# wildminder/ComfyUI-KEEP

Measured on AMD Instinct MI355X. Metric: restored 512x512 face frames/sec, T=20 clip, higher is better.
Workload: dtype f16x3; 1 GPU; 48 independent clips x T=20 x 512x512 per GPU (BASELINE configs[1] clips), KEEP config, synthetic weights seed 0, precision policy x3; clips_per_gpu=48, clip_length=20, parallelism=dp1 over clips, precision_policy=x3

## Files before the change

comfyui-keep_amd/csrc/keep_attn.hip:

```cpp
#include <math.h>
#include <stdlib.h>

#include <type_traits>

#include "keep_common.h"
#include "../../include/keep_cv_hip.h"

static constexpr int KEEP_NT_ATTN_O = 0;


struct AttnP {
  const float* q;
  const float* k;
  const float* v;
  const unsigned short* q16;
  const unsigned short* k16;
  const unsigned short* v16;
  float* o;
  long q_bs, q_ts, q_hs, k_bs, k_ts, k_hs, v_bs, v_ts, v_hs, o_bs, o_ts, o_hs;
  int B, H, Lq, Lk, D, Dv;
  float scale;
  int mode, T, seg_len;
  int img_h, img_w, ksplit, shift, kv_rot, n_img;
  int nslices;
  unsigned flags;
  const _Float16* kv_pack;
  const float* q_amax;
  const float* k_amax;
  const float* v_amax;
};

enum AttnForm {
  ATTN_F32,
  ATTN_BF16,
  ATTN_BF16IN,
  ATTN_X3_NQ8,
  ATTN_X3_NQ16,
  ATTN_X3_NQ0,
  ATTN_X3_PACKED,
  ATTN_X1_PACKED,
  ATTN_X3_SMALL,
  ATTN_X3_TWO_PASS,
  ATTN_X3_SFULL,
  ATTN_X3_SFULL2,
};
struct AttnPlan {
  AttnForm form;
  int waves;
  int dvt;
  bool masked;
  size_t lds;
  int64_t scratch;
  int nq;
  bool win_tables;
};

__device__ __forceinline__ void attn_range_scale(float amax, float& s, float& inv_s) {
  int e = (int)((__float_as_uint(amax) >> 23) & 0xffu);
  if (!(amax > 0.f) || e == 255) {
    s = 1.f;
    inv_s = 1.f;
    return;
  }
  e = e < 15 ? 15 : e;
  s = __uint_as_float((unsigned)(268 - e) << 23);
  inv_s = __uint_as_float((unsigned)(e - 14) << 23);
}

__device__ __forceinline__ void win_shift(const AttnP& p, int wh, int ww, int& sy, int& sx) {
  sy = p.shift > 0 ? wh / 2 : 0;
  sx = p.shift > 0 ? ww / 2 : 0;
}

__device__ __forceinline__ void win_decode(const AttnP& p, int bw, int t, int rot, int& img, int& pix) {
  const int k2 = p.ksplit * p.ksplit;
  img = bw / k2;
  const int widx = bw - img * k2;
  const int wy = widx / p.ksplit, wx = widx - wy * p.ksplit;
  const int wh = p.img_h / p.ksplit, ww = p.img_w / p.ksplit;
  int sy, sx;
  win_shift(p, wh, ww, sy, sx);
  const int ty = (int)(((float)t + 0.5f) * (1.0f / (float)ww)), tx = t - ty * ww;
  int y = wy * wh + ty + sy;
  int x = wx * ww + tx + sx;
  if (y >= p.img_h) y -= p.img_h;
  if (x >= p.img_w) x -= p.img_w;
  pix = y * p.img_w + x;
  if (rot) {
    img += rot;
    if (img >= p.n_img) img -= p.n_img;
  }
}
// ... 416 lines not shown
    l_run = l_run * alpha + lsum;
    m_run = m_new;

#pragma unroll
    for (int r = 0; r < 16; ++r) {
      const int qrow = (r & 3) + 8 * (r >> 2) + 4 * lhi;
      const float ar = __shfl(alpha, qrow);
#pragma unroll
      for (int j = 0; j < DVT; ++j) o[j][r] *= ar;
    }
#pragma unroll
    for (int st = 0; st < 2; ++st) {
      abf16x8 pa;
#pragma unroll
      for (int j = 0; j < 8; ++j) pa[j] = (__bf16)s[st * 8 + j];
#pragma unroll
      for (int j = 0; j < DVT; ++j) {
        const abf16x8 vb = *reinterpret_cast<const abf16x8*>(Vt + (j * 32 + l31) * VP + (st * 2 + lhi) * 8);
        o[j] = __builtin_amdgcn_mfma_f32_32x32x16_bf16(pa, vb, o[j], 0, 0, 0);
      }
    }
  }

  const float inv_l = 1.0f / l_run;
#pragma unroll
  for (int r = 0; r < 16; ++r) {
    const int qrow = (r & 3) + 8 * (r >> 2) + 4 * lhi;
    const float il = __shfl(inv_l, qrow);
    const int t = q0 + wave * 32 + qrow;
    if (t < p.Lq) {
      const long base = q_offset(p, b, t, p.o_bs, p.o_ts) + (long)head * p.o_hs;
#pragma unroll
      for (int j = 0; j < DVT; ++j) {
        const int dv = dv0 + j * 32 + l31;
        if (dv < p.Dv) p.o[base + dv] = o[j][r] * il;
      }
    }
  }
}

template <int WAVES, int DVT>
static int launch_attn_bf16(const AttnP& p, const AttnPlan& pl, hipStream_t st) {
  const int rc = keep_raise_lds_limit<attn_bf16_kernel<WAVES, DVT>>("keep_attention");
  if (rc != KEEP_OK) return rc;
  dim3 grid(cdiv(p.Lq, WAVES * 32), p.H * p.nslices, p.B);
  hipLaunchKernelGGL((attn_bf16_kernel<WAVES, DVT>), grid, dim3(64 * WAVES), pl.lds, st, p);
  KEEP_LAUNCH_CHECK("keep_attention(bf16)");
  return KEEP_OK;
}

typedef _Float16 af16x8 __attribute__((ext_vector_type(8)));
typedef _Float16 af16x4 __attribute__((ext_vector_type(4)));
typedef _Float16 af16x2 __attribute__((ext_vector_type(2)));

template <int WAVES, int DVT, int NQ, bool PACKED = false, bool X1 = false>
__global__ __launch_bounds__(64 * WAVES, ((WAVES == 4 && NQ != 16) ? 2 : 1)) void attn_x3_kernel(AttnP p) {
  static_assert(!X1 || (PACKED && WAVES == 4 && NQ == 8), "the single-fp16 form exists for the packed D = 128 kernel only");
  constexpr bool QREG = NQ > 0;
  constexpr int NQA = QREG ? NQ : 1;
  extern __shared__ __attribute__((aligned(16))) _Float16 smemx[];
  constexpr int DVS = DVT * 32;
  constexpr int NT = 64 * WAVES;
  constexpr int VP = X1 ? 40 : 72;
  constexpr bool PF = (WAVES == 4) && QREG;
  constexpr int KPF = PF ? (32 * 4 * NQA + NT - 1) / NT : 1;
  constexpr int VPF = PF ? (16 * DVS + NT - 1) / NT : 1;
  const int DCMAX = QREG ? 16 * NQA : 128;
  const int DC = p.D < DCMAX ? p.D : DCMAX;
  const int nch = p.D / DC;
  const int QP = (X1 ? DC : 2 * DC) + 8;
  _Float16* Ks = smemx;
  _Float16* Vt = Ks + 32 * QP;
  _Float16* Qs = Vt + DVS * VP;
  const bool tab = PF && p.mode == 2 && p.Lk <= 4096;
  int* tpix = reinterpret_cast<int*>(Qs);
  unsigned* treg = reinterpret_cast<unsigned*>(tpix + ((p.Lk + 31) & ~31));

  const int tid = threadIdx.x;
  const int lane = tid & 63;
  const int wave = tid >> 6;
  const int l31 = lane & 31, lhi = lane >> 5;
  int bx = blockIdx.x, by = blockIdx.y, bz = blockIdx.z;
  {
    const int gx = gridDim.x, gy = gridDim.y, total = gx * gy * gridDim.z;
    const int lid = bx + gx * (by + gy * bz);
    const int qd = total >> 3, rm = total & 7, xcd = lid & 7, slot = lid >> 3;
    const int logical = (xcd < rm ? xcd * (qd + 1) : rm * (qd + 1) + (xcd - rm) * qd) + slot;
    bx = logical % gx;
    const int rest = logical / gx;
    by = rest % gy;
    bz = rest / gy;
  }
  const int b = bz;
  const int head = by / p.nslices;
  const int dv0 = (by - head * p.nslices) * DVS;
  const int q0 = bx * (WAVES * 32);
  const long qh = (long)head * p.q_hs, kh = (long)head * p.k_hs, vh = (long)head * p.v_hs;
  const int g4n = DC >> 2;
  WinCtx wc;
  if (tab) {
    wc = win_ctx(p, b);
    const int ntl = (p.Lk + 31) >> 5;
    unsigned char* treg8 = reinterpret_cast<unsigned char*>(treg + ntl * 4);
    for (int t = tid; t < ntl * 32; t += NT) {
      int pix = 0, region = 0;
      if (t < p.Lk) win_token(p, wc, t, pix, region);
      tpix[t] = pix;
      treg8[t] = (unsigned char)region;
    }
    __syncthreads();
// ... 91 lines not shown
      const int i = tid + u * NT;
      if (i < 32 * g4n) {
        const int row = i / g4n, c = (i - row * g4n) << 2;
        split_store4(kreg[u], sk, Ks + row * QP + c);
      }
    }
  };
  auto v_issue = [&](int kt) {
#pragma unroll
    for (int u = 0; u < VPF; ++u) {
      const int i = tid + u * NT;
      vreg[u][0] = 0.f;
      vreg[u][1] = 0.f;
      if (i < 16 * DVS) {
        const int pair = i / DVS, dv = i - pair * DVS;
        const int t = kt * 32 + pair * 2;
        if (dv0 + dv < p.Dv) {
          if (tab) {
            const long vb = (long)wc.img_kv * p.v_bs + vh + dv0 + dv;
            if (t < p.Lk) vreg[u][0] = p.v[vb + (long)tpix[t] * p.v_ts];
            if (t + 1 < p.Lk) vreg[u][1] = p.v[vb + (long)tpix[t + 1] * p.v_ts];
          } else {
            if (t < p.Lk) vreg[u][0] = p.v[kv_offset(p, b, t, p.v_bs, p.v_ts) + vh + dv0 + dv];
            if (t + 1 < p.Lk) vreg[u][1] = p.v[kv_offset(p, b, t + 1, p.v_bs, p.v_ts) + vh + dv0 + dv];
          }
        }
      }
    }
  };
  auto v_commit = [&]() {
#pragma unroll
    for (int u = 0; u < VPF; ++u) {
      const int i = tid + u * NT;
      if (i < 16 * DVS) {
        const int pair = i / DVS, dv = i - pair * DVS;
        af16x2 hi, lo;
#pragma unroll
        for (int j = 0; j < 2; ++j) {
          const float vs = vreg[u][j] * sv;
          const _Float16 h = (_Float16)vs;
          hi[j] = h;
          lo[j] = (_Float16)(vs - (float)h);
        }
        _Float16* d = Vt + dv * VP + vt_pos(pair * 2);
        *reinterpret_cast<af16x2*>(d) = hi;
        *reinterpret_cast<af16x2*>(d + 32) = lo;
      }
    }
  };

  constexpr int PKK = PACKED ? 32 * ((X1 ? 1 : 2) * 16 * NQA + 8) / 8 : 1;
  constexpr int PKV = PACKED ? DVS * VP / 8 : 1;
  constexpr int PK16 = PKK + PKV;
  constexpr int PKN = PACKED ? (PK16 + NT - 1) / NT : 1;
  uint4 preg[PKN];
  auto pk_issue = [&](int kt) {
    const long tile = ((long)b * p.H + head) * ((p.Lk + 31) >> 5) + kt;
    const uint4* src = reinterpret_cast<const uint4*>(p.kv_pack) + tile * (PKK + p.nslices * PKV);
    const int vs = PKK + (dv0 / DVS) * PKV;
#pragma unroll
    for (int u = 0; u < PKN; ++u) {
      const int i = tid + u * NT;
      preg[u] = make_uint4(0u, 0u, 0u, 0u);
      if (i < PK16) preg[u] = src[i < PKK ? i : vs + (i - PKK)];
    }
  };
  auto pk_commit = [&]() {
#pragma unroll
    for (int u = 0; u < PKN; ++u) {
      const int i = tid + u * NT;
      if (i < PK16) reinterpret_cast<uint4*>(Ks)[i] = preg[u];
    }
  };

  const int my_q = q0 + wave * 32 + l31;
  af16x8 qfh[NQA], qfl[NQA];
  if (QREG) {
    const bool qok = my_q < p.Lq;
    const float* qrow = p.q + (qok ? q_offset(p, b, my_q, p.q_bs, p.q_ts) + qh : 0) + lhi * 8;
#pragma unroll
    for (int d8 = 0; d8 < NQA; ++d8) {
      float4 a = make_float4(0.f, 0.f, 0.f, 0.f), c = a;
      if (qok && d8 * 16 < DC) {
        a = *reinterpret_cast<const float4*>(qrow + d8 * 16);
        c = *reinterpret_cast<const float4*>(qrow + d8 * 16 + 4);
      }
      split8(a, c, sq, qfh[QREG ? d8 : 0], qfl[QREG ? d8 : 0]);
    }
  }
  if (PF) {
    if (PACKED) {
      pk_issue(0);
      pk_commit();
    } else {
      k_issue(0);
      v_issue(0);
      k_commit();
      v_commit();
    }
  }

  int my_region = 0;
  if (p.mode == 2 && p.shift > 0 && my_q < p.Lq) my_region = win_region(p, b, my_q);

  const float qk_scale = p.scale * inv_qk;
  const float qk_scale2 = qk_scale * 1.4426950408889634f;
  float m_run = -INFINITY, l_run = 0.f;
  f32x16 o[DVT];
#pragma unroll
  for (int j = 0; j < DVT; ++j)
#pragma unroll
    for (int r = 0; r < 16; ++r) o[j][r] = 0.f;

  const _Float16* kp = Ks + l31 * QP + lhi * 8;
  const _Float16* qp = Qs + (wave * 32 + l31) * QP + lhi * 8;
  const int ntiles = (p.Lk + 31) / 32;

  for (int kt = 0; kt < ntiles; ++kt) {
    f32x16 s;
#pragma unroll
    for (int r = 0; r < 16; ++r) s[r] = 0.f;
    if (QREG) {
      if (!PF) {
        __syncthreads();
        stage_rows(p.k, p.k_bs, p.k_ts, kh, false, kt * 32, p.Lk, 32, 0, Ks);
        stage_vt(kt);
// ... 52 lines not shown
          if (kr != my_region) val += -100.0f * 1.4426950408889634f;
        }
        if (key >= p.Lk) val = -INFINITY;
        s[r] = val;
        mloc = fmaxf(mloc, val);
      }
    } else {
#pragma unroll
      for (int r = 0; r < 16; ++r) {
        const int key = kt * 32 + (r & 3) + 8 * (r >> 2) + 4 * lhi;
        float val = s[r] * qk_scale;
        if (p.mode == 2 && p.shift > 0 && key < p.Lk) {
          if (win_region(p, b, key) != my_region) val += -100.0f;
        }
        if (key >= p.Lk) val = -INFINITY;
        s[r] = val;
        mloc = fmaxf(mloc, val);
      }
    }
    mloc = fmaxf(mloc, __shfl_xor(mloc, 32));
    const float m_new = fmaxf(m_run, mloc);
    const float alpha = PF ? __builtin_amdgcn_exp2f(m_run - m_new) : expf(m_run - m_new);
    float lsum = 0.f;
#pragma unroll
    for (int r = 0; r < 16; ++r) {
      const float pv = PF ? __builtin_amdgcn_exp2f(s[r] - m_new) : expf(s[r] - m_new);
      s[r] = pv;
      lsum += pv;
    }
    lsum += __shfl_xor(lsum, 32);
    l_run = l_run * alpha + lsum;
    m_run = m_new;

    if (!PF || __builtin_amdgcn_ballot_w64(alpha != 1.0f) != 0ull) {
#pragma unroll
      for (int r = 0; r < 16; ++r) {
        const int qrow = (r & 3) + 8 * (r >> 2) + 4 * lhi;
        const float ar = __shfl(alpha, qrow);
#pragma unroll
        for (int j = 0; j < DVT; ++j) o[j][r] *= ar;
      }
    }
#pragma unroll
    for (int st = 0; st < 2; ++st) {
      af16x8 ph, pl;
#pragma unroll
      for (int j = 0; j < 8; ++j) {
        const _Float16 h = (_Float16)s[st * 8 + j];
        ph[j] = h;
        pl[j] = (_Float16)(s[st * 8 + j] - (float)h);
      }
#pragma unroll
      for (int j = 0; j < DVT; ++j) {
        const _Float16* vrow = Vt + (j * 32 + l31) * VP + (st * 2 + lhi) * 8;
        const af16x8 vh8 = *reinterpret_cast<const af16x8*>(vrow);
        if (!X1) {
          const af16x8 vl8 = *reinterpret_cast<const af16x8*>(vrow + 32);
          o[j] = __builtin_amdgcn_mfma_f32_32x32x16_f16(pl, vh8, o[j], 0, 0, 0);
          o[j] = __builtin_amdgcn_mfma_f32_32x32x16_f16(ph, vl8, o[j], 0, 0, 0);
        }
        o[j] = __builtin_amdgcn_mfma_f32_32x32x16_f16(ph, vh8, o[j], 0, 0, 0);
      }
    }
    if (PF && kt + 1 < ntiles) {
      __syncthreads();
      if (PACKED) {
        pk_commit();
      } else {
        k_commit();
        v_commit();
      }
    }
  }

  const float inv_l = inv_sv / l_run;
#pragma unroll
  for (int r = 0; r < 16; ++r) {
    const int qrow = (r & 3) + 8 * (r >> 2) + 4 * lhi;
    const float il = __shfl(inv_l, qrow);
    const int t = q0 + wave * 32 + qrow;
    if (t < p.Lq) {
      const long base = q_offset(p, b, t, p.o_bs, p.o_ts) + (long)head * p.o_hs;
#pragma unroll
      for (int j = 0; j < DVT; ++j) {
        const int dv = dv0 + j * 32 + l31;
        if (dv >= p.Dv) continue;
        if (KEEP_NT_ATTN_O)
          __builtin_nontemporal_store(o[j][r] * il, p.o + base + dv);
        else
          p.o[base + dv] = o[j][r] * il;
      }
    }
  }
}

template <int DC, int DVS, bool X1 = false>
__global__ __launch_bounds__(256) void attn_pack_kv_x3_kernel(AttnP p, _Float16* out) {
  constexpr int QP = (X1 ? DC : 2 * DC) + 8, VP = X1 ? 40 : 72, PKK = 32 * QP / 8, PKV = DVS * VP / 8;
  __shared__ __attribute__((aligned(16))) _Float16 img[32 * QP + DVS * VP];
  _Float16* Ks = img;
  _Float16* Vt = img + 32 * QP;
  const int tid = threadIdx.x;
  const int kt = blockIdx.x, head = blockIdx.y / p.nslices, slice = blockIdx.y - head * p.nslices, b = blockIdx.z;
  float sk = 1.f, sv = 1.f, tmp;
  if (p.q_amax) {
    attn_range_scale(p.k_amax[b], sk, tmp);
    attn_range_scale(p.v_amax[b], sv, tmp);
  }
  for (int i = tid; i < PKK + PKV; i += 256) reinterpret_cast<uint4*>(img)[i] = make_uint4(0u, 0u, 0u, 0u);
  __syncthreads();
  const long kh = (long)head * p.k_hs, vh = (long)head * p.v_hs;
  if (slice == 0) {
    for (int i = tid; i < 32 * (DC / 4); i += 256) {
      const int row = i / (DC / 4), c = (i - row * (DC / 4)) << 2;
      const int t = kt * 32 + row;
      if (t < p.Lk) {
        const float4 v = *reinterpret_cast<const float4*>(p.k + kv_offset(p, b, t, p.k_bs, p.k_ts) + kh + c);
        const float f[4] = {v.x * sk, v.y * sk, v.z * sk, v.w * sk};
        af16x4 hi, lo;
#pragma unroll
        for (int j = 0; j < 4; ++j) {
          const _Float16 h = (_Float16)f[j];
          hi[j] = h;
          lo[j] = (_Float16)(f[j] - (float)h);
        }
        *reinterpret_cast<af16x4*>(Ks + row * QP + c) = hi;
        if (!X1) *reinterpret_cast<af16x4*>(Ks + row * QP + DC + c) = lo;
      }
    }
  }
  const int dv0 = slice * DVS;
  for (int i = tid; i < 16 * DVS; i += 256) {
    const int pair = i / DVS, dv = i - pair * DVS;
    const int t = kt * 32 + pair * 2;
    float v[2] = {0.f, 0.f};
    if (dv0 + dv < p.Dv) {
      if (t < p.Lk) v[0] = p.v[kv_offset(p, b, t, p.v_bs, p.v_ts) + vh + dv0 + dv];
      if (t + 1 < p.Lk) v[1] = p.v[kv_offset(p, b, t + 1, p.v_bs, p.v_ts) + vh + dv0 + dv];
    }
    af16x2 hi, lo;
#pragma unroll
    for (int j = 0; j < 2; ++j) {
      const float vs = v[j] * sv;
      const _Float16 h = (_Float16)vs;
      hi[j] = h;
      lo[j] = (_Float16)(vs - (float)h);
    }
    _Float16* d = Vt + dv * VP + vt_pos(pair * 2);
    *reinterpret_cast<af16x2*>(d) = hi;
    if (!X1) *reinterpret_cast<af16x2*>(d + 32) = lo;
  }
  __syncthreads();
  uint4* dst = reinterpret_cast<uint4*>(out) + (((long)b * p.H + head) * gridDim.x + kt) * (PKK + p.nslices * PKV);
  if (slice == 0)
    for (int i = tid; i < PKK; i += 256) dst[i] = reinterpret_cast<const uint4*>(img)[i];
  for (int i = tid; i < PKV; i += 256) dst[PKK + slice * PKV + i] = reinterpret_cast<const uint4*>(img)[PKK + i];
}

template <int DVT, int NQ, bool X1 = false>
static int launch_attn_x3_packed(const AttnP& p, const AttnPlan& pl, hipStream_t st) {
  const int ntl = (p.Lk + 31) / 32;
  hipLaunchKernelGGL((attn_pack_kv_x3_kernel<16 * NQ, DVT * 32, X1>), dim3(ntl, p.H * p.nslices, p.B), dim3(256), 0, st, p,
                     const_cast<_Float16*>(p.kv_pack));
  KEEP_LAUNCH_CHECK("keep_attention(x3 pack)");
  const int rc = keep_raise_lds_limit<attn_x3_kernel<4, DVT, NQ, true, X1>>("keep_attention");
  if (rc != KEEP_OK) return rc;
  dim3 grid(cdiv(p.Lq, 128), p.H * p.nslices, p.B);
  hipLaunchKernelGGL((attn_x3_kernel<4, DVT, NQ, true, X1>), grid, dim3(256), pl.lds, st, p);
  KEEP_LAUNCH_CHECK("keep_attention(x3 packed)");
  return KEEP_OK;
}

template <int WAVES, int DVT, int NQ>
static int launch_attn_x3_t(const AttnP& p, const AttnPlan& pl, hipStream_t st) {
  const int rc = keep_raise_lds_limit<attn_x3_kernel<WAVES, DVT, NQ>>("keep_attention");
  if (rc != KEEP_OK) return rc;
  dim3 grid(cdiv(p.Lq, WAVES * 32), p.H * p.nslices, p.B);
  hipLaunchKernelGGL((attn_x3_kernel<WAVES, DVT, NQ>), grid, dim3(64 * WAVES), pl.lds, st, p);
  KEEP_LAUNCH_CHECK("keep_attention(x3)");
  return KEEP_OK;
}

template <int DVT>
__global__ __launch_bounds__(256, 1) void attn_x3_sfull_kernel(AttnP p) {
  extern __shared__ __attribute__((aligned(16))) _Float16 smemx[];
  constexpr int DVS = DVT * 32, NT = 256, VP = 72, DC = 128, QP = 2 * DC + 8, KT2 = 64;
  _Float16* Qs = smemx;
  _Float16* Ks = Qs + 128 * QP;
  _Float16* Vt = Ks + KT2 * QP;
  const int tid = threadIdx.x;
  const int lane = tid & 63;
  const int wave = tid >> 6;
  const int l31 = lane & 31, lhi = lane >> 5;
  const int b = blockIdx.z;
  const int head = blockIdx.y / p.nslices;
  const int dv0 = (blockIdx.y - head * p.nslices) * DVS;
  const int q0 = blockIdx.x * 128;
  const long qh = (long)head * p.q_hs, kh = (long)head * p.k_hs, vh = (long)head * p.v_hs;
  const int nch = p.D / DC;
  const int ntiles = (p.Lk + 31) / 32;
  float sq = 1.f, sk = 1.f, sv = 1.f, inv_qk = 1.f, inv_sv = 1.f;
  if (p.q_amax) {
    float iq, ik;
    attn_range_scale(p.q_amax[b], sq, iq);
    attn_range_scale(p.k_amax[b], sk, ik);
    attn_range_scale(p.v_amax[b], sv, inv_sv);
    inv_qk = iq * ik;
  }
  auto stage_rows = [&](const float* base, long bs, long ts, long hoff, int t0, int tmax, int nrows, int c0, float sc, _Float16* dst) {
    for (int i = tid; i < nrows * (DC / 4); i += NT) {
      const int row = i / (DC / 4), c = (i - row * (DC / 4)) << 2;
      const int t = t0 + row;
      float4 v = make_float4(0.f, 0.f, 0.f, 0.f);
      if (t < tmax) v = *reinterpret_cast<const float4*>(base + (long)b * bs + (long)t * ts + hoff + c0 + c);
      const float f[4] = {v.x * sc, v.y * sc, v.z * sc, v.w * sc};
      af16x4 hi, lo;
#pragma unroll
      for (int j = 0; j < 4; ++j) {
        const _Float16 h = (_Float16)f[j];
        hi[j] = h;
        lo[j] = (_Float16)(f[j] - (float)h);
      }
// ... 962 lines not shown
#pragma unroll 4
    for (int i = lane; i < 32 * C4; i += 64) {
      const int row = i / C4, c4 = (i - row * C4) * 4;
      const long base = ooff[wave * 32 + row];
      if (base >= 0 && dv0 + c4 < p.Dv)
        *reinterpret_cast<float4*>(p.o + base + dv0 + c4) = *reinterpret_cast<const float4*>(ost + row * OP + c4);
    }
    return;
  }
#pragma unroll
  for (int r = 0; r < 16; ++r) {
    const int qrow = (r & 3) + 8 * (r >> 2) + 4 * lhi;
    const float il = __shfl(inv_l, qrow);
    const int t = q0 + wave * 32 + qrow;
    if (t < p.Lq) {
      const long base = tok_q(t, p.o_bs, p.o_ts) + (long)head * p.o_hs;
#pragma unroll
      for (int j = 0; j < DVT; ++j) {
        const int dv = dv0 + j * 32 + l31;
        if (dv < p.Dv) p.o[base + dv] = o[j][r] * il;
      }
    }
  }
}

template <int DVT>
static int launch_attn_bf16in(const AttnP& p, const AttnPlan& pl, hipStream_t st) {
  int rc = keep_raise_lds_limit<attn_bf16in_kernel<DVT, false>>("keep_attention");
  if (rc == KEEP_OK) rc = keep_raise_lds_limit<attn_bf16in_kernel<DVT, true>>("keep_attention");
  if (rc != KEEP_OK) return rc;
  dim3 grid(cdiv(p.Lq, 128), p.H * p.nslices, p.B);
  if (pl.masked)
    hipLaunchKernelGGL((attn_bf16in_kernel<DVT, true>), grid, dim3(256), pl.lds, st, p);
  else
    hipLaunchKernelGGL((attn_bf16in_kernel<DVT, false>), grid, dim3(256), pl.lds, st, p);
  KEEP_LAUNCH_CHECK("keep_attention(bf16 inputs)");
  return KEEP_OK;
}

static int attn_args_in(const keep_attention_args* src, keep_attention_args& a) {
  KEEP_REQUIRE(src != nullptr, "keep_attention: null args");
  const uint32_t sz = src->struct_size;
  if (sz < KEEP_ATTENTION_ARGS_V12_SIZE || sz > sizeof(keep_attention_args) || sz % 8 != 0) {
    keep_set_error("keep_attention: args.struct_size = %u, this library (ABI v%d) accepts %d..%zu -- set it to "
                   "sizeof(keep_attention_args) of the header the caller was built with", sz, KEEP_ABI_VERSION,
                   KEEP_ATTENTION_ARGS_V12_SIZE, sizeof(keep_attention_args));
    return KEEP_EINVAL;
  }
  memset(&a, 0, sizeof(a));
  memcpy(&a, src, sz);
  return KEEP_OK;
}

static int plan_attention(const keep_attention_args& a, int64_t scratch_avail, AttnP& p, AttnPlan& pl) {
  KEEP_REQUIRE(a.B > 0 && a.H > 0 && a.Lq > 0 && a.Lk > 0 && a.D > 0 && a.Dv > 0, "keep_attention: bad dims");
  KEEP_REQUIRE(a.D % 2 == 0 && (a.D <= 128 || a.D % 128 == 0), "keep_attention: D=%d must be even and (<= 128 or a multiple of 128)", a.D);
  KEEP_REQUIRE(a.mode >= 0 && a.mode <= 2, "keep_attention: bad mode %d", a.mode);
  const bool x1 = a.mma == KEEP_MMA_X1 && (a.flags & KEEP_ATTN_X1);
  KEEP_REQUIRE(a.mma != KEEP_MMA_X1 || x1, "keep_attention: KEEP_MMA_X1 has no attention kernel without KEEP_ATTN_X1 (flags), which admits the packed D = Dv = 128 form only");
  KEEP_REQUIRE(a.mma == KEEP_MMA_F32 || a.mma == KEEP_MMA_BF16 || a.mma == KEEP_MMA_X3 || x1, "keep_attention: bad mma %d", a.mma);
  if (a.mode == 1)
    KEEP_REQUIRE(a.T > 0 && a.seg_len > 0 && a.Lk == 2 * a.seg_len && a.B % a.T == 0,
                 "keep_attention: sparse-causal mode needs Lk == 2*seg_len and B %% T == 0");
  if (a.mode == 2) {
    KEEP_REQUIRE(a.ksplit > 0 && a.img_h % a.ksplit == 0 && a.img_w % a.ksplit == 0, "keep_attention: bad window split");
    const int wh = a.img_h / a.ksplit, ww = a.img_w / a.ksplit;
    KEEP_REQUIRE(a.Lq == wh * ww && a.Lk == wh * ww, "keep_attention: window mode needs Lq == Lk == window size");
    KEEP_REQUIRE(a.n_img > 0 && a.B == a.n_img * a.ksplit * a.ksplit, "keep_attention: B != n_img*ksplit^2");
    KEEP_REQUIRE(a.shift == 0 || a.shift == wh / 2, "keep_attention: shift=%d must be 0 or img_h/ksplit/2 = %d", a.shift, wh / 2);
    KEEP_REQUIRE(a.kv_rot >= 0 && a.kv_rot < a.n_img, "keep_attention: bad kv_rot");
    KEEP_REQUIRE((long)a.img_h * a.img_w <= 65536, "keep_attention: window mode supports maps of at most 65536 tokens");
  }
#define ATTN_X1_ADMITS(cond, ...)    \
  do {                               \
    if (!(cond)) {                   \
      keep_set_error(__VA_ARGS__);   \
      return KEEP_EUNSUP;            \
    }                                \
  } while (0)
  if (x1) ATTN_X1_ADMITS(!a.q_amax && !a.k_amax && !a.v_amax, "keep_attention: KEEP_MMA_X1 takes no q/k/v_amax range probes (normalised operands only)");
  KEEP_REQUIRE((!a.q_amax && !a.k_amax && !a.v_amax) || (a.q_amax && a.k_amax && a.v_amax && a.mode == 0 && a.mma == KEEP_MMA_X3),
               "keep_attention: q/k/v_amax come together, with KEEP_MMA_X3 and mode 0 only");
  p.flags = a.flags;
  p.q = (const float*)a.q; p.k = (const float*)a.k; p.v = (const float*)a.v; p.o = a.o;
  p.q16 = (const unsigned short*)a.q; p.k16 = (const unsigned short*)a.k; p.v16 = (const unsigned short*)a.v;
  p.q_bs = a.q_bs; p.q_ts = a.q_ts; p.q_hs = a.q_hs;
  p.k_bs = a.k_bs; p.k_ts = a.k_ts; p.k_hs = a.k_hs;
  p.v_bs = a.v_bs; p.v_ts = a.v_ts; p.v_hs = a.v_hs;
  p.o_bs = a.o_bs; p.o_ts = a.o_ts; p.o_hs = a.o_hs;
  p.B = a.B; p.H = a.H; p.Lq = a.Lq; p.Lk = a.Lk; p.D = a.D; p.Dv = a.Dv;
  p.scale = a.scale; p.mode = a.mode; p.T = a.T; p.seg_len = a.seg_len;
  p.img_h = a.img_h; p.img_w = a.img_w; p.ksplit = a.ksplit; p.shift = a.shift; p.kv_rot = a.kv_rot;
  p.n_img = a.n_img;
  p.q_amax = a.q_amax; p.k_amax = a.k_amax; p.v_amax = a.v_amax;
  p.kv_pack = nullptr;
  const int dvt = a.Dv <= 32 ? 1 : (a.Dv <= 64 ? 2 : 4);
  p.nslices = cdiv(a.Dv, dvt * 32);
  pl = AttnPlan{ATTN_F32, a.Lq <= 32 ? 1 : 4, dvt, false, 0, 0, 0, false};

  auto rows16 = [](const void* base, int64_t bs, int64_t ts, int64_t hs, int n) {
    return bs % n == 0 && ts % n == 0 && hs % n == 0 && (uintptr_t)base % 16 == 0;
  };
  const int DC = a.D < 128 ? a.D : 128;
  const size_t ntl = (size_t)(a.Lk + 31) / 32;
  const size_t win_tables = ntl * 32 * 4 + ntl * 16 + ntl * 32;

  if (x1) {
    ATTN_X1_ADMITS(a.in_dtype == KEEP_F32, "keep_attention: KEEP_MMA_X1 needs fp32 q / k / v (in_dtype KEEP_F32)");
    ATTN_X1_ADMITS(a.mode == 0 || a.mode == 2, "keep_attention: KEEP_MMA_X1 covers mode 0 and mode 2, not mode %d", a.mode);
    ATTN_X1_ADMITS(a.D == 128 && a.Dv == 128, "keep_attention: KEEP_MMA_X1 covers D = Dv = 128 only (D=%d Dv=%d)", a.D, a.Dv);
    ATTN_X1_ADMITS(a.Lq >= 256, "keep_attention: KEEP_MMA_X1 covers Lq >= 256 only (Lq=%d): the packed form", a.Lq);
    ATTN_X1_ADMITS(rows16(a.q, a.q_bs, a.q_ts, a.q_hs, 4) && rows16(a.k, a.k_bs, a.k_ts, a.k_hs, 4) && rows16(a.v, a.v_bs, a.v_ts, a.v_hs, 4),
                   "keep_attention: KEEP_MMA_X1 needs 16-byte aligned q / k / v rows");
    ATTN_X1_ADMITS(!(a.flags & KEEP_ATTN_NO_PACK), "keep_attention: KEEP_MMA_X1 has the packed form only (KEEP_ATTN_NO_PACK is set)");
    const int64_t need = (int64_t)a.B * a.H * (int64_t)ntl * ((32 * (a.D + 8) + p.nslices * dvt * 32 * 40) * 2L);
    ATTN_X1_ADMITS(scratch_avail >= need, "keep_attention: KEEP_MMA_X1 needs a 16-byte aligned workspace of %lld bytes (keep_attention_workspace_bytes), got %lld",
                   (long long)need, (long long)scratch_avail);
    pl.form = ATTN_X1_PACKED;
    pl.waves = 4;
    pl.nq = 8;
    pl.win_tables = a.mode == 2 && a.Lk <= 4096;
    pl.lds = (size_t)(32 * (a.D + 8) + dvt * 32 * 40) * 2 + (pl.win_tables ? win_tables : 0);
    pl.scratch = need;
    return KEEP_OK;
  }
#undef ATTN_X1_ADMITS
  if (a.in_dtype == KEEP_BF16) {
    const bool ok = a.mma == KEEP_MMA_BF16 && a.D % 16 == 0 && a.Dv % 8 == 0 && rows16(a.q, a.q_bs, a.q_ts, a.q_hs, 8) &&
                    rows16(a.k, a.k_bs, a.k_ts, a.k_hs, 8) && rows16(a.v, a.v_bs, a.v_ts, a.v_hs, 8);
    KEEP_REQUIRE(ok, "keep_attention: bf16 inputs need KEEP_MMA_BF16, D %% 16 == 0, Dv %% 8 == 0 and 16-byte aligned rows");
    const size_t operands = (size_t)((128 + 64) * (DC + 8) + dvt * 32 * 72) * 2;
    const size_t staging = (size_t)4 * 32 * (dvt * 32 + 4) * 4;
    pl.form = ATTN_BF16IN;
    pl.waves = 4;
    pl.masked = a.mode == 2 && a.shift > 0;
    pl.lds = (128 + 3 * 64 + 3 * 64) * sizeof(long) + 3 * 16 * sizeof(unsigned long long) + (operands > staging ? operands : staging);
    return KEEP_OK;
  }
  const bool qk16 = a.D % 16 == 0 && rows16(a.q, a.q_bs, a.q_ts, a.q_hs, 4) && rows16(a.k, a.k_bs, a.k_ts, a.k_hs, 4);
  if (a.mma == KEEP_MMA_BF16) {
    KEEP_REQUIRE(qk16, "keep_attention: KEEP_MMA_BF16 needs D %% 16 == 0 and 16-byte aligned q/k rows");
    pl.form = ATTN_BF16;
    pl.lds = (size_t)((pl.waves * 32 + 32) * (DC + 8) + dvt * 32 * 40) * 2;
    return KEEP_OK;
  }
  if (a.mma != KEEP_MMA_X3 || !qk16 || (a.flags & KEEP_ATTN_NO_X3)) {
    pl.lds = (size_t)((pl.waves * 32 + 32) * (DC + 1) + 32 * dvt * 32) * sizeof(float);
    return KEEP_OK;
  }

  const bool v16 = rows16(a.v, a.v_bs, a.v_ts, a.v_hs, 4), o16 = rows16(a.o, a.o_bs, a.o_ts, a.o_hs, 4);
  auto x3_lds = [&](int waves, int nq) {
    const int dc = nq == 0 ? 128 : (a.D < 16 * nq ? a.D : 16 * nq);
    const size_t lds = (size_t)(((nq ? 0 : waves * 32) + 32) * (2 * dc + 8) + dvt * 32 * 72) * 2;
    pl.nq = nq;
    pl.win_tables = waves == 4 && nq && a.mode == 2 && a.Lk <= 4096;
    return lds + (pl.win_tables ? win_tables : 0);
  };
  if (a.mode == 0 && a.D == 64 && a.Dv == 64 && a.Lk <= 256 && a.Lq >= 64 && v16 && o16 && !(a.flags & KEEP_ATTN_NO_SMALL)) {
// ... 20 lines not shown
  if (a.D <= 128) {
    pl.form = ATTN_X3_NQ8;
    pl.lds = x3_lds(pl.waves, 8);
    return KEEP_OK;
  }
  pl.waves = 4;
  if (a.D <= 256) {
    pl.form = ATTN_X3_NQ16;
    pl.lds = x3_lds(4, 16);
  } else if (a.mode == 0 && a.D == 512 && a.Lk <= 256 && a.Dv <= 512 && a.Dv % 4 == 0 && v16 && !(a.flags & KEEP_ATTN_NO_SFULL2)) {
    pl.form = ATTN_X3_SFULL2;
    pl.lds = (size_t)4 * (2 * 32 * (2 * 128 + 8)) * 2 + 4 * 1024 * 4;
  } else if (a.mode == 0 && a.Lk <= 256 && a.D % 128 == 0) {
    pl.form = ATTN_X3_SFULL;
    pl.lds = (size_t)((128 + 64) * (2 * 128 + 8) + dvt * 32 * 72) * 2;
  } else {
    pl.form = ATTN_X3_NQ0;
    pl.lds = x3_lds(4, 0);
  }
  return KEEP_OK;
}

template <class F>
static int with_dvt(int dvt, F f) {
  if (dvt == 1) return f(std::integral_constant<int, 1>{});
  if (dvt == 2) return f(std::integral_constant<int, 2>{});
  return f(std::integral_constant<int, 4>{});
}

extern "C" int32_t keep_sizeof_attention_args(void) { return (int32_t)sizeof(keep_attention_args); }

extern "C" int64_t keep_attention_workspace_bytes(const keep_attention_args* a_in) {
  keep_attention_args a;
  AttnP p;
  AttnPlan pl;
  if (attn_args_in(a_in, a) != KEEP_OK) return 0;
  const int rc = plan_attention(a, INT64_MAX, p, pl);
  if (rc != KEEP_OK) return (rc == KEEP_EUNSUP && a.mma == KEEP_MMA_X1) ? -1 : 0;
  return pl.scratch;
}

static void attn_plan_kernel_name(const AttnPlan& pl, char* out, size_t n) {
  const int dvs = pl.dvt * 32;
  switch (pl.form) {
    case ATTN_F32: snprintf(out, n, "attn_f32_kernel<%d, %d>", pl.waves, pl.dvt); return;
    case ATTN_BF16: snprintf(out, n, "attn_bf16_kernel<%d, %d>", pl.waves, pl.dvt); return;
    case ATTN_BF16IN: snprintf(out, n, "attn_bf16in_kernel<%d, %s>", pl.dvt, pl.masked ? "true" : "false"); return;
    case ATTN_X3_NQ8:
    case ATTN_X3_NQ16:
    case ATTN_X3_NQ0: snprintf(out, n, "attn_x3_kernel<%d, %d, %d, false, false>", pl.waves, pl.dvt, pl.nq); return;
    case ATTN_X3_PACKED:
      snprintf(out, n, "attn_pack_kv_x3_kernel<%d, %d, false> + attn_x3_kernel<4, %d, %d, true, false>", 16 * pl.nq, dvs, pl.dvt, pl.nq);
      return;
    case ATTN_X1_PACKED:
      snprintf(out, n, "attn_pack_kv_x3_kernel<%d, %d, true> + attn_x3_kernel<4, %d, %d, true, true>", 16 * pl.nq, dvs, pl.dvt, pl.nq);
      return;
    case ATTN_X3_SMALL: snprintf(out, n, "attn_x3_small_kernel"); return;
    case ATTN_X3_TWO_PASS: snprintf(out, n, "attn_scores_x3l_kernel + attn_pv_x3l_kernel"); return;
    case ATTN_X3_SFULL: snprintf(out, n, "attn_x3_sfull_kernel<%d>", pl.dvt); return;
    case ATTN_X3_SFULL2: snprintf(out, n, "attn_x3_sfull2_kernel"); return;
  }
  snprintf(out, n, "?");
}

extern "C" int32_t keep_attention_plan(const keep_attention_args* a_in, keep_attention_plan_out* out) {
  KEEP_REQUIRE(out != nullptr, "keep_attention_plan: null out");
  memset(out, 0, sizeof(*out));
  keep_attention_args a;
  const int rc_in = attn_args_in(a_in, a);
  if (rc_in != KEEP_OK) return rc_in;
  AttnP p;
  AttnPlan pl;
  const bool ws_ok = a.workspace && (uintptr_t)a.workspace % 16 == 0;
  const int rc = plan_attention(a, ws_ok ? a.workspace_bytes : 0, p, pl);
  if (rc != KEEP_OK) return rc;
  out->waves = pl.waves;
  out->dvt = pl.dvt;
  out->nslices = p.nslices;
  out->masked = pl.masked;
  out->win_tables = pl.win_tables;
  out->lds_bytes = (int64_t)pl.lds;
  AttnP p_all;
  AttnPlan pl_all;
  out->scratch_bytes = plan_attention(a, INT64_MAX, p_all, pl_all) == KEEP_OK ? pl_all.scratch : 0;
  attn_plan_kernel_name(pl, out->kernel, sizeof(out->kernel));
  return KEEP_OK;
}

extern "C" int32_t keep_attention(const keep_attention_args* a_in, void* stream) {
  keep_attention_args a;
  const int rc_in = attn_args_in(a_in, a);
  if (rc_in != KEEP_OK) return rc_in;
  KEEP_REQUIRE(a.q && a.k && a.v && a.o, "keep_attention: null tensor pointer");
  AttnP p;
  AttnPlan pl;
  const bool ws_ok = a.workspace && (uintptr_t)a.workspace % 16 == 0;
  const int rc = plan_attention(a, ws_ok ? a.workspace_bytes : 0, p, pl);
  if (rc != KEEP_OK) return rc;
  hipStream_t st = (hipStream_t)stream;
  const bool one_wave = pl.waves == 1;
  switch (pl.form) {
    case ATTN_F32:
      return with_dvt(pl.dvt, [&](auto dvt) {
        return one_wave ? launch_attn<1, decltype(dvt)::value>(p, pl, st) : launch_attn<4, decltype(dvt)::value>(p, pl, st);
      });
    case ATTN_BF16:
      return with_dvt(pl.dvt, [&](auto dvt) {
        return one_wave ? launch_attn_bf16<1, decltype(dvt)::value>(p, pl, st) : launch_attn_bf16<4, decltype(dvt)::value>(p, pl, st);
      });
    case ATTN_BF16IN:
      return with_dvt(pl.dvt, [&](auto dvt) { return launch_attn_bf16in<decltype(dvt)::value>(p, pl, st); });
    case ATTN_X3_NQ8:
      return with_dvt(pl.dvt, [&](auto dvt) {
        return one_wave ? launch_attn_x3_t<1, decltype(dvt)::value, 8>(p, pl, st) : launch_attn_x3_t<4, decltype(dvt)::value, 8>(p, pl, st);
      });
    case ATTN_X3_NQ16:
      return with_dvt(pl.dvt, [&](auto dvt) { return launch_attn_x3_t<4, decltype(dvt)::value, 16>(p, pl, st); });
    case ATTN_X3_NQ0:
      return with_dvt(pl.dvt, [&](auto dvt) { return launch_attn_x3_t<4, decltype(dvt)::value, 0>(p, pl, st); });
    case ATTN_X3_PACKED:
      p.kv_pack = (const _Float16*)a.workspace;
      return with_dvt(pl.dvt, [&](auto dvt) {
        return pl.nq == 8 ? launch_attn_x3_packed<decltype(dvt)::value, 8>(p, pl, st) : launch_attn_x3_packed<decltype(dvt)::value, 16>(p, pl, st);
      });
    case ATTN_X1_PACKED:
      p.kv_pack = (const _Float16*)a.workspace;
      return launch_attn_x3_packed<4, 8, true>(p, pl, st);
    case ATTN_X3_SMALL:
      return launch_attn_x3_small(p, st);
    case ATTN_X3_TWO_PASS:
      return launch_attn_x3_two_pass(p, (float*)a.workspace, st);
    case ATTN_X3_SFULL:
      return with_dvt(pl.dvt, [&](auto dvt) { return launch_attn_x3_sfull<decltype(dvt)::value>(p, pl, st); });
    case ATTN_X3_SFULL2:
      return launch_attn_x3_sfull2(p, pl, st);
  }
  keep_set_error("keep_attention: no kernel form planned");
  return KEEP_EINVAL;
}

#define MLP_C 128
__global__ __launch_bounds__(256, 2) void gm_mlp_kernel(const float* __restrict__ xa, const float* __restrict__ xb,
                                                        const unsigned short* __restrict__ w0,
                                                        const unsigned short* __restrict__ w2, float* __restrict__ out,
                                                        long M) {
  constexpr int K1 = 2 * MLP_C, HID = 8 * MLP_C, HC = 64;
  constexpr int P0 = K1 + 8;
  constexpr int P2 = HC + 8;
  constexpr int OP = MLP_C + 4;
  constexpr int OPER_B = (HC * P0 + MLP_C * P2) * 2;
  constexpr int STAGE_B = 4 * 32 * OP * 4;
  __shared__ __attribute__((aligned(16))) unsigned char lds_raw[OPER_B > STAGE_B ? OPER_B : STAGE_B];
  __bf16* W0s = reinterpret_cast<__bf16*>(lds_raw);
  __bf16* W2s = W0s + HC * P0;

  const int tid = threadIdx.x;
  const int lane = tid & 63;
  const int wave = tid >> 6;
  const int l31 = lane & 31, lhi = lane >> 5;
  const long m0 = (long)blockIdx.x * 128;
  const long my_tok = m0 + wave * 32 + l31;

  abf16x8 xf[16];
#pragma unroll
  for (int ks = 0; ks < 16; ++ks) {
    const int c = ks * 16 + lhi * 8;
    float4 v0 = make_float4(0.f, 0.f, 0.f, 0.f), v1 = v0;
    if (my_tok < M) {
      const float* src = (c < MLP_C ? xa + my_tok * MLP_C + c : xb + my_tok * MLP_C + (c - MLP_C));
      v0 = *reinterpret_cast<const float4*>(src);
      v1 = *reinterpret_cast<const float4*>(src + 4);
    }
    xf[ks][0] = (__bf16)v0.x; xf[ks][1] = (__bf16)v0.y; xf[ks][2] = (__bf16)v0.z; xf[ks][3] = (__bf16)v0.w;
    xf[ks][4] = (__bf16)v1.x; xf[ks][5] = (__bf16)v1.y; xf[ks][6] = (__bf16)v1.z; xf[ks][7] = (__bf16)v1.w;
  }

  uint4 p00, p01, p02, p03, p04, p05, p06, p07, p20, p21, p22, p23;
#define MLP_P0(X) X(0, p00) X(1, p01) X(2, p02) X(3, p03) X(4, p04) X(5, p05) X(6, p06) X(7, p07)
#define MLP_P2(X) X(0, p20) X(1, p21) X(2, p22) X(3, p23)
#define MLP_LD0(U, R) R = *reinterpret_cast<const uint4*>(w0 + (long)(hc_n * HC + ((tid + (U) * 256) >> 5)) * K1 + (((tid + (U) * 256) & 31) << 3));
#define MLP_LD2(U, R) R = *reinterpret_cast<const uint4*>(w2 + (long)((tid + (U) * 256) >> 3) * HID + hc_n * HC + (((tid + (U) * 256) & 7) << 3));
#define MLP_ST0(U, R) *reinterpret_cast<uint4*>(W0s + ((tid + (U) * 256) >> 5) * P0 + (((tid + (U) * 256) & 31) << 3)) = R;
#define MLP_ST2(U, R)                                                                                   \
  {                                                                                                     \
    const int h8 = ((tid + (U) * 256) & 7) << 3;                                                        \
    uint2* d = reinterpret_cast<uint2*>(W2s + ((tid + (U) * 256) >> 3) * P2 + (h8 >> 5) * 32 + vt_pos(h8 & 31)); \
    d[0] = make_uint2(R.x, R.y);                                                                        \
    d[2] = make_uint2(R.z, R.w);                                                                        \
  }

  f32x16 o[4];
#pragma unroll
// ... 221 lines not shown
```

comfyui-keep_amd/csrc/keep_conv.hip:

```cpp
#include <cxxabi.h>
#include <stdlib.h>

#include <string>

#include "keep_conv_common.h"
#include "../../include/keep_cv_hip.h"

template <int WGM, int WGN, int TM, int TN, bool PLAIN = false>
__global__ __launch_bounds__(256) void conv_f32_kernel(ConvP p) {
  constexpr int BM = WGM * TM * 32;
  constexpr int BN = WGN * TN * 32;
  constexpr int LDA = BM + 2;
  constexpr int LDB = BN + 2;
  constexpr int A_TPR = 256 / BM;
  constexpr int A_CPT = BK / A_TPR;
  constexpr int B_TPR = 256 / BN;
  constexpr int B_CPT = BK / B_TPR;
  static_assert(WGM * WGN == 4, "4 waves");
  static_assert(A_TPR >= 1 && B_TPR >= 1 && A_CPT >= 1 && B_CPT >= 1, "tile config");

  constexpr int MAIN_F = 2 * BK * (LDA + LDB);
  constexpr int EPI_F = 4 * (TM * 32) * (TN * 32 + 4);
  __shared__ __attribute__((aligned(16))) float smem_f[MAIN_F > EPI_F ? MAIN_F : EPI_F];
  float(*As)[BK * LDA] = reinterpret_cast<float(*)[BK * LDA]>(smem_f);
// ... 1553 lines not shown
  KEEP_REQUIRE(a->N > 0 && a->H > 0 && a->W > 0 && a->Cin > 0 && a->Cout > 0 && a->KH > 0 && a->KW > 0 &&
                   a->stride > 0 && a->Ho > 0 && a->Wo > 0,
               "keep_conv2d: non-positive dimension");
  KEEP_REQUIRE(a->in_ld >= (a->in2 ? a->in2_cin1 : a->Cin) && a->out_ld >= a->Cout, "keep_conv2d: ld smaller than channel count");
  if (a->in2 && a->mma != KEEP_MMA_X3) {
    keep_set_error("keep_conv2d: in2 (K-concatenated input) is a KEEP_MMA_X3 feature");
    return KEEP_EUNSUP;
  }
  KEEP_REQUIRE((a->pro_scale == nullptr) == (a->pro_shift == nullptr), "keep_conv2d: pro_scale/pro_shift must pair");
  KEEP_REQUIRE(!a->aux || a->residual, "keep_conv2d: aux epilogue requires residual");
  KEEP_REQUIRE(!a->residual || a->res_ld >= a->Cout, "keep_conv2d: res_ld smaller than Cout");
  KEEP_REQUIRE(a->split_k >= 0, "keep_conv2d: split_k must be >= 0 (0 = let the library choose)");
  const int Hv = a->upsample ? 2 * a->H : a->H, Wv = a->upsample ? 2 * a->W : a->W;
  KEEP_REQUIRE((long)(a->Ho - 1) * a->stride - a->pad_t < Hv && (long)(a->Wo - 1) * a->stride - a->pad_l < Wv,
               "keep_conv2d: output extent %dx%d inconsistent with input %dx%d", a->Ho, a->Wo, Hv, Wv);
  KEEP_REQUIRE(a->mma == KEEP_MMA_F32 || a->mma == KEEP_MMA_BF16 || a->mma == KEEP_MMA_X3 || a->mma == KEEP_MMA_X1, "keep_conv2d: bad mma %d", a->mma);
  KEEP_REQUIRE(a->upsample == 0 || a->upsample == 1 ||
                   (a->upsample == KEEP_UPSAMPLE_X2_PHASES &&
                    (a->mma == KEEP_MMA_X3 || (a->mma == KEEP_MMA_X1 && (a->flags & KEEP_CONV_X1_UP2)))),
               "keep_conv2d: upsample must be 0, 1 or KEEP_UPSAMPLE_X2_PHASES (KEEP_MMA_X3, or KEEP_MMA_X1 with KEEP_CONV_X1_UP2), got %d", a->upsample);
  KEEP_REQUIRE(a->pad_mode == KEEP_PAD_ZERO || a->pad_mode == KEEP_PAD_REFLECT, "keep_conv2d: bad pad_mode %d", a->pad_mode);
  if (a->pad_mode == KEEP_PAD_REFLECT) {
    if (a->mma == KEEP_MMA_BF16 || a->dtype != KEEP_F32 || a->pad_t != a->pad_l || a->pad_t >= Hv || a->pad_t >= Wv ||
        a->pad_t != a->KH / 2 || a->KH != a->KW) {
      keep_set_error("keep_conv2d: KEEP_PAD_REFLECT needs fp32 tensors, KEEP_MMA_F32 / KEEP_MMA_X3, a square odd kernel and pad_t == pad_l == KH/2 < min(H, W)");
      return KEEP_EUNSUP;
    }
  }
  KEEP_REQUIRE((long)a->N * a->Ho * a->Wo < (1L << 31), "keep_conv2d: M too large");
  if (a->ln_gamma && (a->mma != KEEP_MMA_X3 || a->KH != 1 || a->KW != 1 || a->stride != 1 || a->upsample)) {
    keep_set_error("keep_conv2d: ln_gamma (LayerNorm epilogue) is a feature of the KEEP_MMA_X3 GEMM form (1x1, stride 1)");
    return KEEP_EUNSUP;
  }
  return KEEP_OK;
}

static void fill_conv_params(const keep_conv2d_args* a, ConvP& p) {
  p.in = (const float*)a->in;
  p.w = a->weight;
  p.wb = (const unsigned short*)a->weight_bf16;
  p.wx3 = (const unsigned short*)a->weight_x3;
  p.acc_scale = a->x3_acc_scale;
  p.in_amax = (a->mma == KEEP_MMA_X3 && a->pro_act != KEEP_PRO_NONE) ? nullptr : a->x3_in_amax;
  p.in2 = (const float*)a->in2;
  p.cin1 = a->in2_cin1;
  p.out_amax = nullptr;
  p.reflect = a->pad_mode == KEEP_PAD_REFLECT ? 1 : 0;
  p.tile_cols = 0;
  p.reverse = 0;
  p.ln_gamma = a->ln_gamma;
  p.ln_beta = a->ln_beta;
  p.ln_eps = a->ln_eps;
  p.kslice_steps = 0;
  p.bias = a->bias;
  p.out = (float*)a->out;
  p.pro_scale = a->pro_scale;
  p.pro_shift = a->pro_shift;
  p.res = (const float*)a->residual;
  p.aux = (const float*)a->aux;
  p.ws = a->workspace;
  p.N = a->N; p.H = a->H; p.W = a->W; p.Cin = a->Cin; p.Cout = a->Cout; p.KH = a->KH; p.KW = a->KW;
  p.stride = a->stride; p.pad_t = a->pad_t; p.pad_l = a->pad_l; p.Ho = a->Ho; p.Wo = a->Wo;
  p.in_ld = a->in_ld; p.out_ld = a->out_ld; p.res_ld = a->res_ld;
  p.upsample = a->upsample; p.pro_act = a->pro_act; p.epi_act = a->epi_act; p.aux_w = a->aux_w;
  p.M = (int)((long)a->N * a->Ho * a->Wo);
  p.cchunks = (a->Cin + BK - 1) / BK;
  p.nsteps = a->KH * a->KW * p.cchunks;
  p.in_bf16 = (a->dtype == KEEP_BF16) ? 1 : 0;
  p.fast = (a->mma == KEEP_MMA_BF16 || ((a->mma == KEEP_MMA_X3 || a->mma == KEEP_MMA_X1) && !(a->flags & KEEP_CONV_X3_EXACT_ACT))) ? 1 : 0;
  p.out_bf16 = (a->out_dtype == KEEP_BF16) ? 1 : 0;
  p.vec_ok = (a->Cin % 4 == 0 && a->in_ld % 4 == 0 && ((uintptr_t)a->in % 16 == 0)) ? 1 : 0;
  p.vec_epi = (a->Cout % 4 == 0 && a->out_ld % 4 == 0 && (uintptr_t)a->out % 16 == 0 &&
               (!a->residual || (a->res_ld % 4 == 0 && (uintptr_t)a->residual % 16 == 0)) &&
               (!a->aux || (uintptr_t)a->aux % 16 == 0) && (!a->bias || (uintptr_t)a->bias % 16 == 0) &&
               (!a->workspace || (uintptr_t)a->workspace % 16 == 0)) ? 1 : 0;
  p.flatk = 0;
  p.flatk_f32 = 0;
  p.stats = a->stats_out;
  p.stats_P = a->stats_P;
}

struct ConvGeom {
  long M;
  int ncb;
  bool no_pro, is33s1, same_size, tileable, pro_al, epi_al, reflect;
};

static ConvGeom conv_geom(const keep_conv2d_args* a) {
  ConvGeom g;
  g.M = a->mma == KEEP_MMA_BF16 ? (long)a->N * a->Ho * a->Wo : plan_ref_images(a) * (long)a->Ho * a->Wo;
  g.ncb = (a->Cout + 63) / 64;
  g.no_pro = !a->pro_scale && a->pro_act == KEEP_PRO_NONE;
  g.is33s1 = a->KH == 3 && a->KW == 3 && a->stride == 1 && a->pad_t == 1 && a->pad_l == 1;
  g.same_size = a->Ho == (a->upsample ? 2 * a->H : a->H) && a->Wo == (a->upsample ? 2 * a->W : a->W);
  g.tileable = (a->Ho % 8 == 0 && a->Wo % 32 == 0) || (a->Ho % 16 == 0 && a->Wo % 16 == 0);
  g.pro_al = !a->pro_scale || ((uintptr_t)a->pro_scale % 16 == 0 && (uintptr_t)a->pro_shift % 16 == 0);
  g.epi_al = (a->out_ld % 4 == 0) && ((uintptr_t)a->out % 16 == 0) &&
             (!a->residual || (a->res_ld % 4 == 0 && (uintptr_t)a->residual % 16 == 0)) &&
             (!a->aux || (uintptr_t)a->aux % 16 == 0) && (!a->bias || (uintptr_t)a->bias % 16 == 0);
  g.reflect = a->pad_mode == KEEP_PAD_REFLECT;
  return g;
}

static int pick_split_k(const keep_conv2d_args* a, int auto_split, int cap) {
  const int s = a->split_k > 0 ? a->split_k : auto_split;
  return s > cap ? cap : s;
// ... 237 lines not shown
      const int auto_split = (a->out_dtype == KEEP_BF16 || waves >= kTargetWaves) ? 1
                             : (int)max(1L, min(min((long)kTargetWaves / waves, (long)a->Cin / 64), 16L));
      pl.split_k = pick_split_k(a, auto_split, a->Cin / 32);
      pl.stats_rows = g.no_pro ? 64 : 256;
      return KEEP_OK;
    }
  }
  if (p.in_bf16) {
    keep_set_error("keep_conv2d: bf16 input tensors are only accepted by the 3x3 stride-1 halo path "
                   "(Cin%%32, Cout%%32, tileable map, no prologue)");
    return KEEP_EUNSUP;
  }
  pl.path = PATH_GATHER_BF16;
  pl.tile = a->Cout <= 32 ? 0 : gather_tile(a, g);
  pl.stats_rows = pl.tile == 1 ? 64 : 128;
  p.flatk = (a->Cin < 8 && g.no_pro) ? 1 : 0;
  pl.plain = !p.flatk && p.vec_ok && g.no_pro && !a->upsample && (a->Cin % 8 == 0) && !(a->flags & KEEP_CONV_NO_PLAIN);
  pl.bk256 = a->bk256 && !p.flatk && pl.tile == 1;
  const int steps = pl.bk256 ? a->KH * a->KW * ((a->Cin + 255) / 256)
                    : (p.flatk ? (a->KH * a->KW * a->Cin + BK16 - 1) / BK16 : a->KH * a->KW * ((a->Cin + BK16 - 1) / BK16));
  const int auto_split = a->out_dtype == KEEP_BF16 ? 1 : gather_auto_split(gather_waves(pl.tile, g.M, a->Cout), steps, pl.bk256 ? SPLIT_BK256 : SPLIT_HALF);
  pl.out_bf16_ok = (p.vec_epi && !a->residual) ? 1 : 0;
  pl.split_k = pick_split_k(a, auto_split, steps);
  return KEEP_OK;
}

static int plan_form(const keep_conv2d_args* a, ConvP& p, const ConvGeom& g, ConvPlan& pl) {
  if (a->Cout <= 4 && g.is33s1 && !g.reflect && !a->upsample && a->dtype == KEEP_F32 && a->out_dtype != KEEP_BF16 && a->Cin % SC_CH == 0 &&
      a->in_ld % 4 == 0 && (uintptr_t)a->in % 16 == 0 && a->Ho == a->H && a->Wo == a->W && a->Ho % SC_TH == 0 &&
      a->Wo % SC_TW == 0 && !a->residual && !a->aux && a->split_k <= 1 && g.pro_al && !(a->flags & KEEP_CONV_NO_COUT4)) {
    pl.path = PATH_COUT4;
    pl.split_k = 1;
    return KEEP_OK;
  }
  if (a->mma == KEEP_MMA_BF16 && g.is33s1 && !a->upsample && a->Cin <= 3 && a->Cout % 4 == 0 && a->Cout >= 32 && a->dtype == KEEP_F32 &&
      a->out_dtype != KEEP_BF16 && a->Ho == a->H && a->Wo == a->W && a->Ho % 8 == 0 && a->Wo % 32 == 0 && g.no_pro && !a->residual &&
      !a->aux && a->split_k <= 1 && a->out_ld % 4 == 0 && (uintptr_t)a->out % 16 == 0 && (!a->bias || (uintptr_t)a->bias % 16 == 0) &&
      !(a->flags & KEEP_CONV_NO_C3)) {
    pl.path = PATH_C3;
    pl.split_k = 1;
    pl.stats_rows = 64;
    return KEEP_OK;
  }
  if (a->mma == KEEP_MMA_X1) return plan_x1(a, p, g, pl);
  if (a->mma == KEEP_MMA_BF16) return plan_bf16(a, p, g, pl);
  if (a->mma == KEEP_MMA_X3) {
    bool to_f32;
    const int rc = plan_x3(a, p, g, pl, to_f32);
    if (!to_f32) return rc;
  }
  return plan_f32(a, p, g, pl);
}

static int plan_conv(const keep_conv2d_args* a, ConvP& p, ConvPlan& pl) {
  memset(&pl, 0, sizeof(pl));
  fill_conv_params(a, p);
  pl.wide = (a->Ho % 8 == 0 && a->Wo % 32 == 0);
  const int rc = plan_form(a, p, conv_geom(a), pl);
  if (rc == KEEP_OK) plan_kernel_name(a, pl);
  return rc;
}

static int conv_args_in(const keep_conv2d_args* src, keep_conv2d_args& a) {
  KEEP_REQUIRE(src != nullptr, "keep_conv2d: null args");
  const uint32_t sz = src->struct_size;
  if (sz < KEEP_CONV2D_ARGS_V12_SIZE || sz > sizeof(keep_conv2d_args) || sz % 8 != 0) {
    keep_set_error("keep_conv2d: args.struct_size = %u, this library (ABI v%d) accepts %d..%zu -- set it to sizeof(keep_conv2d_args) "
                   "of the header the caller was built with", sz, KEEP_ABI_VERSION, KEEP_CONV2D_ARGS_V12_SIZE, sizeof(keep_conv2d_args));
    return KEEP_EINVAL;
  }
  memset(&a, 0, sizeof(a));
  memcpy(&a, src, sz);
  return KEEP_OK;
}

extern "C" int32_t keep_sizeof_conv2d_args(void) { return (int32_t)sizeof(keep_conv2d_args); }

static int conv_prelude(const keep_conv2d_args* a_in, bool launch, keep_conv2d_args& a, ConvP& p, ConvPlan& pl) {
  int rc = conv_args_in(a_in, a);
  if (rc != KEEP_OK) return rc;
  rc = validate_conv(&a);
  if (rc != KEEP_OK) return rc;
  if (launch) {
    KEEP_REQUIRE(a.in && a.weight && a.out, "keep_conv2d: null tensor pointer");
    KEEP_REQUIRE((uintptr_t)a.weight % 16 == 0, "keep_conv2d: weight pointer must be 16-byte aligned");
    KEEP_REQUIRE(!a.pro_scale || ((uintptr_t)a.pro_scale % 16 == 0 && (uintptr_t)a.pro_shift % 16 == 0),
                 "keep_conv2d: pro_scale/pro_shift must be 16-byte aligned");
  }
  return plan_conv(&a, p, pl);
}

extern "C" int32_t keep_conv2d_plan(const keep_conv2d_args* a_in, keep_conv2d_plan_out* out) {
  KEEP_REQUIRE(out != nullptr, "keep_conv2d_plan: null output");
  keep_conv2d_args a_local;
  ConvP p;
  ConvPlan pl;
  const int rc = conv_prelude(a_in, false, a_local, p, pl);
  if (rc != KEEP_OK) return rc;
  const keep_conv2d_args* a = &a_local;
  memset(out, 0, sizeof(*out));
  const long hw_o = (long)a->Ho * a->Wo;
  out->split_k = pl.split_k;
  out->workspace_bytes = pl.split_k > 1 ? (int64_t)pl.split_k * a->N * hw_o * a->Cout * 4 : 0;
  out->stats_rows = (pl.split_k == 1 && pl.stats_rows > 0 && hw_o % pl.stats_rows == 0 && a->out_ld == a->Cout) ? pl.stats_rows : 0;
  out->stats_P = out->stats_rows ? (int32_t)(hw_o / out->stats_rows) : 0;
  out->wants_bf16_input = pl.wants_bf16_input;
  out->out_bf16_ok = pl.out_bf16_ok;
  out->out_amax_ok = pl.amax_ok ? 1 : 0;
  out->path = (int32_t)pl.path;
  strncpy(out->kernel, pl.kernel, sizeof(out->kernel) - 1);
  return KEEP_OK;
}

void keep_conv_trace_add(ConvTrace* tr, const char* mangled) {
  int status = 0;
  char* full = abi::__cxa_demangle(mangled, nullptr, nullptr, &status);
  std::string name = (status == 0 && full) ? full : mangled;
  free(full);
  int depth = 0;
  for (size_t i = 0; i < name.size(); ++i) {
    if (name[i] == '<') ++depth;
    if (name[i] == '>') --depth;
    if (name[i] == '(' && depth == 0) {
      name.resize(i);
      break;
    }
  }
  if (name.compare(0, 5, "void ") == 0) name.erase(0, 5);
  const int n = snprintf(tr->buf + tr->len, (size_t)(tr->cap - tr->len), "%s%s", tr->len ? " + " : "", name.c_str());
  if (n < 0 || n >= tr->cap - tr->len) {
    tr->overflow = true;
    tr->buf[tr->len] = 0;
    return;
  }
  tr->len += n;
  ++tr->count;
}

static int conv_launch(const keep_conv2d_args* a_in, void* stream, ConvTrace* tr) {
  keep_conv2d_args a_local;
  ConvP p;
  ConvPlan pl;
  int rc = conv_prelude(a_in, true, a_local, p, pl);
  if (rc != KEEP_OK) return rc;
  const keep_conv2d_args* a = &a_local;
  if (pl.path == PATH_NEEDS_PRENORM) {
    keep_set_error("keep_conv2d: a bf16 input with a prologue must go through keep_norm_act_bf16 first (keep_conv2d_plan: wants_bf16_input)");
    return KEEP_EUNSUP;
  }
  p.split_k = pl.split_k;
  KEEP_REQUIRE(p.split_k == 1 || a->workspace, "keep_conv2d: split_k>1 requires a workspace (keep_conv2d_plan gives its size)");
  const long M = p.M;
  const long hw_o = (long)a->Ho * a->Wo;
  if (p.stats) {
    KEEP_REQUIRE(p.split_k == 1, "keep_conv2d: stats_out requires split_k == 1");
    KEEP_REQUIRE(pl.stats_rows > 0 && hw_o % pl.stats_rows == 0 && a->stats_P == hw_o / pl.stats_rows,
                 "keep_conv2d: stats_P=%d must equal Ho*Wo/%d (keep_conv2d_plan)", a->stats_P, pl.stats_rows);
  }
  hipStream_t st = (hipStream_t)stream;
  if (a->x3_out_amax) {
    KEEP_REQUIRE(pl.amax_ok, "keep_conv2d: x3_out_amax is not available for this call (keep_conv2d_plan: out_amax_ok)");
    if (!a->x3_out_amax_zeroed) {
      KEEP_CONV_LAUNCH(tr, dim3(cdiv(a->N, 256)), dim3(256), st, (reinterpret_cast<unsigned*>(a->x3_out_amax), a->N), zero_u32_kernel);
      KEEP_CONV_LAUNCH_CHECK(tr, "keep_conv2d(zero x3_out_amax)");
    }
    p.out_amax = reinterpret_cast<unsigned*>(a->x3_out_amax);
  }
  if (p.out_bf16)
    KEEP_REQUIRE(p.vec_epi && p.split_k == 1 && !a->residual,
                 "keep_conv2d: bf16 output needs Cout/out_ld %% 4 == 0, aligned pointers, split_k == 1, no residual");
  dim3 block(256);
  const int tw = pl.wide ? 32 : 16, th = 256 / tw;
  const int tiles_x = a->Wo / tw, tiles_y = a->Ho / th, ncb = (a->Cout + 63) / 64;
  const int n_cu = conv_num_cu(tr);
  switch (pl.path) {
    case PATH_COUT4: {
      dim3 grid((a->Ho / SC_TH) * (a->Wo / SC_TW), a->N);
      KEEP_CONV_LAUNCH(tr, grid, block, st, (p), conv3x3_cout4_kernel);
      KEEP_CONV_LAUNCH_CHECK(tr, "keep_conv2d(cout<=4)");
      return KEEP_OK;
    }
    case PATH_C3: {
      const int tx = a->Wo / 32, ty = a->Ho / 8;
      const int n_items = a->N * tx * ty * ncb;
      KEEP_CONV_LAUNCH(tr, dim3(persistent_grid(n_items, n_cu)), block, st, (p, tx, ty, ncb, n_items), conv3x3_c3_kernel);
      KEEP_CONV_LAUNCH_CHECK(tr, "keep_conv2d(Cin<=3)");
      return KEEP_OK;
    }
    case PATH_C3_X3:
      rc = keep_conv2d_x3_c3(a, p, st, tr);
      if (rc != KEEP_OK) return rc;
      break;
    case PATH_HALO_X3:
      rc = keep_conv2d_x3_halo(a, p, pl, st, tr);
      if (rc != KEEP_OK) return rc;
      break;
// ... 68 lines not shown
        else
          KEEP_CONV_LAUNCH(tr, grid, block, st, (p), conv_bf16_kernel<2, 2, 1, 1, 64, 1>);
      } else {
        dim3 grid(cdiv(M, 128), cdiv(a->Cout, 128), p.split_k);
        if (pl.plain)
          KEEP_CONV_LAUNCH(tr, grid, block, st, (p), conv_bf16_kernel<2, 2, 2, 2, 64, 1, true>);
        else
          KEEP_CONV_LAUNCH(tr, grid, block, st, (p), conv_bf16_kernel<2, 2, 2, 2, 64, 1>);
      }
      KEEP_CONV_LAUNCH_CHECK(tr, "keep_conv2d(gather bf16)");
      break;
    }
    case PATH_GATHER_F32: {
      if (pl.tile == 0) {
        dim3 grid(cdiv(M, 128), cdiv(a->Cout, 32), p.split_k);
        KEEP_CONV_LAUNCH(tr, grid, block, st, (p), conv_f32_kernel<4, 1, 1, 1>);
      } else if (pl.tile == 1) {
        dim3 grid(cdiv(M, 64), cdiv(a->Cout, 64), p.split_k);
        if (pl.plain)
          KEEP_CONV_LAUNCH(tr, grid, block, st, (p), conv_f32_kernel<2, 2, 1, 1, true>);
        else
          KEEP_CONV_LAUNCH(tr, grid, block, st, (p), conv_f32_kernel<2, 2, 1, 1>);
      } else {
        dim3 grid(cdiv(M, 128), cdiv(a->Cout, 128), p.split_k);
        if (pl.plain)
          KEEP_CONV_LAUNCH(tr, grid, block, st, (p), conv_f32_kernel<2, 2, 2, 2, true>);
        else
          KEEP_CONV_LAUNCH(tr, grid, block, st, (p), conv_f32_kernel<2, 2, 2, 2>);
      }
      KEEP_CONV_LAUNCH_CHECK(tr, "keep_conv2d(gather f32)");
      break;
    }
    case PATH_NEEDS_PRENORM: break;
  }
  if (p.split_k > 1) {
    const long total = M * a->Cout;
    if (p.vec_epi) {
      int blocks = cdiv(total / 4, 256);
      if (blocks > 4096) blocks = 4096;
      KEEP_CONV_LAUNCH(tr, dim3(blocks), dim3(256), st, (p), conv_splitk_reduce4_kernel);
      KEEP_CONV_LAUNCH_CHECK(tr, "keep_conv2d(split-K reduce)");
      return KEEP_OK;
    }
    int blocks = cdiv(total, 256);
    if (blocks > 4096) blocks = 4096;
    KEEP_CONV_LAUNCH(tr, dim3(blocks), dim3(256), st, (p), conv_splitk_reduce_kernel);
    KEEP_CONV_LAUNCH_CHECK(tr, "keep_conv2d(split-K reduce)");
  }
  return KEEP_OK;
}

extern "C" int32_t keep_conv2d(const keep_conv2d_args* a_in, void* stream) { return conv_launch(a_in, stream, nullptr); }

extern "C" int32_t keep_conv2d_launch_plan(const keep_conv2d_args* a_in, keep_conv2d_launch_plan_out* out) {
  KEEP_REQUIRE(out != nullptr, "keep_conv2d_launch_plan: null output");
  memset(out, 0, sizeof(*out));
  ConvTrace tr = {out->kernels, (int)sizeof(out->kernels), 0, 0, false};
  const int rc = conv_launch(a_in, nullptr, &tr);
  if (rc == KEEP_OK && tr.overflow) {
    memset(out, 0, sizeof(*out));
    keep_set_error("keep_conv2d_launch_plan: the kernel names do not fit keep_conv2d_launch_plan_out.kernels");
    return KEEP_EINVAL;
  }
  if (rc != KEEP_OK) memset(out, 0, sizeof(*out));
  else out->n_kernels = tr.count;
  return rc;
}
```

comfyui-keep_amd/csrc/keep_conv_common.h:

```cpp
#pragma once
#include <type_traits>

#include "keep_common.h"

#define BK 16

static constexpr int KEEP_LD_AUX_XS = 0;
static constexpr int KEEP_LD_AUX_RES = 0;
static constexpr int KEEP_LD_AUX_GEMM_A1 = 0;
static constexpr int KEEP_NT_C3 = 0;
static constexpr int KEEP_ST_AUX_XS = 2;
static constexpr int KEEP_ST_AUX_HALO = 2;
static constexpr int KEEP_ST_AUX_GEMM = 2;

struct ConvP {
  const float* in;
  const float* w;
  const unsigned short* wb;
  const float* bias;
  float* out;
  const float* pro_scale;
  const float* pro_shift;
  const float* res;
  const float* aux;
  float* ws;
  int N, H, W, Cin, Cout, KH, KW, stride, pad_t, pad_l, Ho, Wo;
  int in_ld, out_ld, res_ld;
  int upsample, pro_act, epi_act;
  float aux_w;
  int split_k;
  int M;
  int cchunks;
  int nsteps;
  int vec_ok;
  int in_bf16;
  int fast;
  float* stats;
  int stats_P;
  int out_bf16;
  int vec_epi;
  int flatk;
  int flatk_f32;
  const unsigned short* wx3;
  float acc_scale;
  const float* in_amax;
  const float* in2;
  int cin1;
  unsigned* out_amax;
  int reflect;
  int tile_cols;
  int reverse;
  const float* ln_gamma;
  const float* ln_beta;
  float ln_eps;
  int kslice_steps;
};


#define KEEP_REFLECT(IY, IX, HV, WV)                                   \
  if (p.reflect) {                                                     \
    IY = IY < 0 ? -IY : (IY >= (HV) ? 2 * (HV) - 2 - IY : IY);          \
    IX = IX < 0 ? -IX : (IX >= (WV) ? 2 * (WV) - 2 - IX : IX);          \
  }

static __global__ void zero_u32_kernel(unsigned* p, int n) {
  const int i = blockIdx.x * blockDim.x + threadIdx.x;
  if (i < n) p[i] = 0u;
}

__device__ __forceinline__ void wave_amax_commit(unsigned* dst, float m) {
  unsigned b = __float_as_uint(m);
#pragma unroll
  for (int o = 32; o > 0; o >>= 1) b = max(b, (unsigned)__shfl_xor((int)b, o));
  if ((threadIdx.x & 63) == 0 && b > *reinterpret_cast<volatile unsigned*>(dst)) atomicMax(dst, b);
}

__device__ __forceinline__ void x3_range_scale(float amax, float& s, float& inv_s) {
  int e = (int)((__float_as_uint(amax) >> 23) & 0xffu);
  if (!(amax > 0.f) || e == 255) {
    s = 1.f;
    inv_s = 1.f;
    return;
  }
  e = e < 15 ? 15 : e;
  s = __uint_as_float((unsigned)(268 - e) << 23);
  inv_s = __uint_as_float((unsigned)(e - 14) << 23);
}

__device__ __forceinline__ float epilogue_one(const ConvP& p, float v, long m, int co) {
  if (p.bias) v += p.bias[co];
  v = p.fast ? act_apply_fast(v, p.epi_act) : act_apply(v, p.epi_act);
  if (p.res) {
    float r = p.res[m * p.res_ld + co];
    if (p.aux) {
      float a = p.aux[m * (long)p.Cout + co];
      v = r + p.aux_w * (r * a + v);
    } else {
      v = v + r;
    }
  }
  return v;
}

template <int WGM, int WGN, int TN>
__device__ __forceinline__ void emit_tile_stats(const ConvP& p, float (*red)[2], const float (&cs)[TN], const float (&css)[TN],
                                                int wm, int wn, int lane, int n_img, int p_idx, int n0) {
  const int l31 = lane & 31;
#pragma unroll
// ... 323 lines not shown
```

comfyui-keep_amd/csrc/keep_conv_x3.hip:

```cpp
#include <stdlib.h>

#include "keep_conv_common.h"

typedef _Float16 f16x8 __attribute__((ext_vector_type(8)));
typedef _Float16 f16x4 __attribute__((ext_vector_type(4)));
typedef unsigned int u32x4 __attribute__((ext_vector_type(4)));
typedef float f32x2 __attribute__((ext_vector_type(2)));
typedef _Float16 f16x2 __attribute__((ext_vector_type(2)));

__device__ __forceinline__ void split4(const float (&v)[4], f16x4& hi, f16x4& lo) {
#pragma unroll
  for (int j = 0; j < 4; ++j) {
    const _Float16 h = (_Float16)v[j];
    hi[j] = h;
    lo[j] = (_Float16)(v[j] - (float)h);
  }
}

template <int PRO, bool FAST>
__device__ __forceinline__ float pro_x3(float v) {
  return FAST ? pro_apply_x3(v, PRO) : pro_apply(v, PRO);
}

typedef unsigned int u32x2 __attribute__((ext_vector_type(2)));
// ... 419 lines not shown
      if (nxt.ch_begin < nxt.ch_end) fetch(nxt.ch_begin);
    }
    const float amx = p.res ? epilogue_t(cur, cur_inv, cur_bias, std::true_type{}) : epilogue_t(cur, cur_inv, cur_bias, std::false_type{});
    if (p.out_amax) {
      if (cur.n != amax_n) {
        amax_n = cur.n;
        amax_run = 0.f;
      }
      if (__builtin_amdgcn_ballot_w64(amx > amax_run) != 0ull) {
        unsigned b = __float_as_uint(amx);
#pragma unroll
        for (int o = 32; o > 0; o >>= 1) b = max(b, (unsigned)__shfl_xor((int)b, o));
        unsigned* dst = p.out_amax + cur.n;
        unsigned seen = b;
        if (lane == 0) {
          seen = *reinterpret_cast<volatile unsigned*>(dst);
          if (b > seen) atomicMax(dst, b);
        }
        seen = max(b, (unsigned)__builtin_amdgcn_readfirstlane((int)seen));
        amax_run = fmaxf(amax_run, __uint_as_float(seen));
      }
    }
    if (!has_next) break;
    __syncthreads();
    item = next_item;
    cur = nxt;
  }
}

template <int WGM, int WGN, int TM, int TN, bool SIMPLE>
__device__ __forceinline__ void x3_gather_epilogue(const ConvP& p, f32x16 (&acc)[TM][TN], float* lds, long m0, int n0, int wm,
                                                   int wn, int lane, int wave, int z) {
  constexpr int WR = TM * 32, WC = TN * 32, EP = WC + 4, BM = WGM * WR;
  constexpr int LPR = WC / 4, RPI = 64 / LPR;
  const int l31 = lane & 31, lhi = lane >> 5;
  float* et = lds + wave * WR * EP;
#pragma unroll
  for (int i = 0; i < TM; ++i)
#pragma unroll
    for (int j = 0; j < TN; ++j)
#pragma unroll
      for (int r = 0; r < 16; ++r) et[(i * 32 + (r & 3) + 8 * (r >> 2) + 4 * lhi) * EP + j * 32 + l31] = acc[i][j][r];
  __builtin_amdgcn_s_waitcnt(0xc07f);
  auto make_rsrc = [&](const void* ptr, int bytes) {
    const unsigned long long b = (unsigned long long)ptr;
    const unsigned lo = __builtin_amdgcn_readfirstlane((unsigned)b), hi = __builtin_amdgcn_readfirstlane((unsigned)(b >> 32));
    return __builtin_amdgcn_make_buffer_rsrc((void*)(((unsigned long long)hi << 32) | lo), 0, bytes, 0x00020000);
  };
  const int c4 = (lane % LPR) * 4, prow = lane / LPR;
  const int co = n0 + wn * WC + c4;
  const bool cok = co < p.Cout;
  const int row0 = wm * WR + prow;
  const __amdgpu_buffer_rsrc_t out_rsrc = make_rsrc(p.out + m0 * p.out_ld, BM * p.out_ld * 4);
  const int v_out = cok ? (row0 * p.out_ld + co) * 4 : (int)0x80000000;
  __amdgpu_buffer_rsrc_t res_rsrc = out_rsrc, aux_rsrc = out_rsrc, ws_rsrc = out_rsrc;
  int v_res = (int)0x80000000, v_aux = (int)0x80000000, v_ws = (int)0x80000000;
  if (p.res) {
    res_rsrc = make_rsrc(p.res + m0 * p.res_ld, BM * p.res_ld * 4);
    v_res = cok ? (row0 * p.res_ld + co) * 4 : (int)0x80000000;
    if (!SIMPLE && p.aux) {
      aux_rsrc = make_rsrc(p.aux + m0 * p.Cout, BM * p.Cout * 4);
      v_aux = cok ? (row0 * p.Cout + co) * 4 : (int)0x80000000;
    }
  }
  if (!SIMPLE && p.split_k > 1) {
    ws_rsrc = make_rsrc(p.ws + ((long)z * p.M + m0) * p.Cout, BM * p.Cout * 4);
    v_ws = cok ? (row0 * p.Cout + co) * 4 : (int)0x80000000;
  }
  float s4[4] = {0.f, 0.f, 0.f, 0.f}, ss4[4] = {0.f, 0.f, 0.f, 0.f};
  float amx = 0.f;
  float4 bias4 = make_float4(0.f, 0.f, 0.f, 0.f);
  if (p.bias && p.split_k == 1 && cok) bias4 = *reinterpret_cast<const float4*>(p.bias + co);
  constexpr bool LN_OK = SIMPLE && WGN == 1 && TN == 4;
  const bool ln = LN_OK && p.ln_gamma != nullptr;
  float4 lng = make_float4(1.f, 1.f, 1.f, 1.f), lnb = make_float4(0.f, 0.f, 0.f, 0.f);
  if (ln) {
    lng = *reinterpret_cast<const float4*>(p.ln_gamma + c4);
    lnb = *reinterpret_cast<const float4*>(p.ln_beta + c4);
  }
  constexpr int NIT = WR / RPI, GRP = NIT < 8 ? NIT : 8;
  constexpr int UNR = SIMPLE ? GRP : 4;
  u32x4 rpre[SIMPLE ? GRP : 1];
#pragma unroll UNR
  for (int it = 0; it < NIT; ++it) {
    if (SIMPLE && p.res && (it % GRP) == 0) {
#pragma unroll
      for (int u = 0; u < GRP; ++u) rpre[u] = __builtin_amdgcn_raw_buffer_load_b128(res_rsrc, v_res + (it + u) * RPI * p.res_ld * 4, 0, 0);
    }
    const int px = it * RPI + prow;
    const float4 v = *reinterpret_cast<const float4*>(et + px * EP + c4);
    if (!SIMPLE && p.split_k > 1) {
      u32x4 o;
      o.x = __float_as_uint(v.x); o.y = __float_as_uint(v.y); o.z = __float_as_uint(v.z); o.w = __float_as_uint(v.w);
      __builtin_amdgcn_raw_buffer_store_b128(o, ws_rsrc, v_ws + it * RPI * p.Cout * 4, 0, 0);
      continue;
    }
    float e[4] = {v.x + bias4.x, v.y + bias4.y, v.z + bias4.z, v.w + bias4.w};
    if (!SIMPLE) {
#pragma unroll
      for (int q = 0; q < 4; ++q) e[q] = p.fast ? act_apply_fast(e[q], p.epi_act) : act_apply(e[q], p.epi_act);
    }
    if (LN_OK && ln) {
      float sm = (e[0] + e[1]) + (e[2] + e[3]);
#pragma unroll
      for (int o = 1; o < 32; o <<= 1) sm += __shfl_xor(sm, o);
      const float mean = sm * (1.0f / 128.0f);
      const float d[4] = {e[0] - mean, e[1] - mean, e[2] - mean, e[3] - mean};
      float qq = (d[0] * d[0] + d[1] * d[1]) + (d[2] * d[2] + d[3] * d[3]);
#pragma unroll
      for (int o = 1; o < 32; o <<= 1) qq += __shfl_xor(qq, o);
      const float rstd = 1.0f / sqrtf(qq * (1.0f / 128.0f) + p.ln_eps);
      e[0] = d[0] * rstd * lng.x + lnb.x;
      e[1] = d[1] * rstd * lng.y + lnb.y;
      e[2] = d[2] * rstd * lng.z + lnb.z;
      e[3] = d[3] * rstd * lng.w + lnb.w;
    }
    if (p.res) {
      const u32x4 r4 = SIMPLE ? rpre[SIMPLE ? it % GRP : 0] : __builtin_amdgcn_raw_buffer_load_b128(res_rsrc, v_res + it * RPI * p.res_ld * 4, 0, 0);
      const float rr[4] = {__uint_as_float(r4.x), __uint_as_float(r4.y), __uint_as_float(r4.z), __uint_as_float(r4.w)};
      if (!SIMPLE && p.aux) {
        const u32x4 a4 = __builtin_amdgcn_raw_buffer_load_b128(aux_rsrc, v_aux + it * RPI * p.Cout * 4, 0, 0);
        const float aa[4] = {__uint_as_float(a4.x), __uint_as_float(a4.y), __uint_as_float(a4.z), __uint_as_float(a4.w)};
#pragma unroll
        for (int q = 0; q < 4; ++q) e[q] = rr[q] + p.aux_w * (rr[q] * aa[q] + e[q]);
      } else {
#pragma unroll
        for (int q = 0; q < 4; ++q) e[q] += rr[q];
      }
    }
    {
      u32x4 o;
      o.x = __float_as_uint(e[0]); o.y = __float_as_uint(e[1]); o.z = __float_as_uint(e[2]); o.w = __float_as_uint(e[3]);
      __builtin_amdgcn_raw_buffer_store_b128(o, out_rsrc, v_out + it * RPI * p.out_ld * 4, 0, KEEP_ST_AUX_GEMM);
    }
#pragma unroll
    for (int q = 0; q < 4; ++q) {
      s4[q] += e[q];
      ss4[q] += e[q] * e[q];
      amx = fmaxf(amx, fabsf(e[q]));
    }
  }
  if (p.out_amax) wave_amax_commit(p.out_amax + (int)((m0 + wm * WR) / ((long)p.Ho * p.Wo)), amx);
  if (p.stats) {
#pragma unroll
    for (int q = 0; q < 4; ++q) {
      if (LPR == 8) {
        s4[q] += __shfl_xor(s4[q], 8);
        ss4[q] += __shfl_xor(ss4[q], 8);
      }
      s4[q] = xor32_sum(xor16_sum(s4[q]));
      ss4[q] = xor32_sum(xor16_sum(ss4[q]));
    }
    __syncthreads();
    float* red = lds;
    if (lane < LPR) {
#pragma unroll
      for (int q = 0; q < 4; ++q) {
        red[(wave * WC + c4 + q) * 2 + 0] = s4[q];
        red[(wave * WC + c4 + q) * 2 + 1] = ss4[q];
      }
    }
    __syncthreads();
    constexpr int BNc = WGN * WC;
    const int hw_o = p.Ho * p.Wo;
    const int n_img = (int)(m0 / hw_o), p_idx = (int)((m0 % hw_o) / BM);
    for (int c = threadIdx.x; c < BNc; c += 256) {
      const int wn_c = c / WC, rem = c - wn_c * WC;
      float a = 0.f, b2 = 0.f;
#pragma unroll
      for (int mm = 0; mm < WGM; ++mm) {
        a += red[((mm * WGN + wn_c) * WC + rem) * 2 + 0];
        b2 += red[((mm * WGN + wn_c) * WC + rem) * 2 + 1];
      }
      if (n0 + c < p.Cout) {
        float* dst = p.stats + (((long)n_img * p.stats_P + p_idx) * p.Cout + n0 + c) * 2;
        dst[0] = a;
        dst[1] = b2;
      }
    }
  }
}

#define XBK 32
// ... 816 lines not shown
```

comfyui-keep_amd/engine/hiplib.py:

```python
import ctypes as C
import os

import torch

_HERE = os.path.dirname(os.path.abspath(__file__))
LIB_PATH = os.environ.get('KEEP_HIP_LIB') or os.path.join(os.path.dirname(_HERE), 'csrc', 'libkeep_hip.so')
ABI_VERSION = 23

F32, BF16 = 0, 1
MMA_F32, MMA_BF16, MMA_X3, MMA_X1 = 0, 1, 2, 3
PRO_NONE, PRO_SWISH, PRO_RELU = 0, 1, 2
ACT_NONE, ACT_RELU, ACT_LRELU02, ACT_GELU, ACT_SIGMOID, ACT_LRELU01, ACT_SILU = 0, 1, 2, 3, 4, 5, 6
PAD_ZERO, PAD_REFLECT = 0, 1
UPSAMPLE_X2_PHASES = 2
(CONV_NO_COUT4, CONV_NO_C3, CONV_NO_HALO_F32, CONV_NO_HALO_X3, CONV_NO_GATHER_X3, CONV_NO_PLAIN, CONV_NO_FLATK_F32,
 CONV_SMALL_TILES, CONV_X3_EXACT_ACT, CONV_NO_STREAM, CONV_NO_GEMM_LAT, CONV_GEMM_LAT_WAVES, CONV_GEMM_LAT_TILES, CONV_NO_SMALL_PARTIALS) = (1 << i for i in range(14))
CONV_X1_HALO16 = 1 << 15
CONV_X1_UP2 = 1 << 16
CONV_X1_GEMM = 1 << 14
ATTN_NO_PACK, ATTN_NO_SFULL2, ATTN_NO_X3, ATTN_NO_SMALL, ATTN_NO_TWO_PASS = 1, 2, 4, 8, 16
ATTN_X1 = 1 << 5

_vp, _i32, _i64, _f32, _u32 = C.c_void_p, C.c_int32, C.c_int64, C.c_float, C.c_uint32
STATUS_NONFINITE_LOGITS, STATUS_NONFINITE_TENSOR = 1, 2
# ... 60 lines not shown
    'keep_nchw_to_nhwc': [_vp, _vp, _i32, _i32, _i32, _i32, _vp],
    'keep_rgb_s2d': [_vp, _vp, _i32, _i32, _i32, _vp],
    'keep_nhwc_to_nchw': [_vp, _vp, _i32, _i32, _i32, _vp],
    'keep_add_bcast': [_vp, _vp, _vp, _i64, _i64, _f32, _vp],
    'keep_concat2': [_vp, _vp, _vp, _i64, _i32, _i32, _i32, _vp],
    'keep_tensor2img': [_vp, _vp, _i64, _vp],
    'keep_img2tensor': [_vp, _vp, _i64, _vp],
    'keep_bgr_u8_to_comfy': [_vp, _vp, _i64, _vp],
    'keep_comfy_to_bgr_u8': [_vp, _vp, _i64, _vp],
    'keep_channel_argmax': [_vp, _vp, _i64, _i32, _i32, _vp],
    'keep_maxpool3s2': [_vp, _vp, _i32, _i32, _i32, _i32, _vp],
    'keep_dwconv3x3': [_vp, _vp, _vp, _vp, _i32, _i32, _i32, _i32, _i32, _i32, _vp],
    'keep_maxpool2d': [_vp, _vp, _i32, _i32, _i32, _i32, _i32, _i32, _i32, _i32, _i32, _i32, _i32, _vp],
    'keep_slice_copy': [_vp, _vp, _i32, _i32, _i32, _i32, _i32, _i32, _i32, _vp],
    'keep_channel_shuffle2': [_vp, _vp, _vp, _i64, _i32, _i32, _i32, _vp],
    'keep_yolo_decode': [_vp, _vp, _i32, _i32, _i32, _f32, _vp, _i32, _i32, _vp],
    'keep_yolo_letterbox_u8': [_vp, _vp, _i32, _i32, _i32, _i32, _i32, _i32, _i32, _i32, _i32, _i32, _vp],
    'keep_yolo_select': [_vp, _vp, _vp, _i32, _i32, _i32, _f32, _vp],
    'keep_upsample_add': [_vp, _vp, _vp, _i32, _i32, _i32, _i32, _i32, _i32, _vp],
    'keep_act_inplace': [_vp, _i64, _i32, _vp],
    'keep_retina_decode': [_vp, _vp, _vp, _vp, _i32, _i32, _i32, _f32, _f32, _f32, _f32, _f32, _vp],
    'keep_retina_nms': [_vp, _vp, _vp, _vp, _i32, _i32, _f32, _vp],
    'keep_retina_nms_ordered': [_vp, _vp, _vp, _vp, _vp, _i32, _i32, _f32, _vp],
    'keep_sep_filter': [_vp, _vp, _vp, _vp, _vp, _i32, _i32, _i32, _vp, _i32, _vp],
    'keep_u8_to_f32': [_vp, _vp, _i64, _vp],
    'keep_f32_round_u8': [_vp, _vp, _i64, _vp],
    'keep_warp_affine_u8': [_vp, _i32, _i32, _vp, _i32, _i32, _vp, _i32, _i32, _i32, _vp],
    'keep_warp_ones': [_vp, _i32, _i32, _i32, _i32, _vp, _vp],
    'keep_draw_box': [_vp, _i32, _i32, _i32, _i32, _i32, _vp, _i32, _i32, _i32, _i32, _vp],
    'keep_erode_rect': [_vp, _vp, _vp, _i32, _i32, _i32, _vp],
    'keep_paste_face': [_vp, _i32, _i32, _vp, _vp, _i32, _i32, _vp, _i32, _i32, _i32, _i32, _i32, _vp],
    'keep_lanczos4_tables': [_i32, _i32, _vp, _vp],
    'keep_resize_lanczos4_u8': [_vp, _vp, _i32, _i32, _i32, _i32, _i32, _vp, _vp, _vp, _vp, _vp],
}
EXPORTED_SYMBOLS = ['keep_abi_version', 'keep_last_error', 'keep_device_ok', 'keep_attention_workspace_bytes',
                    'keep_sizeof_conv2d_args', 'keep_sizeof_attention_args'] + list(_SIGNATURES)

CV_ABI_VERSION = 1
_CV_SIGNATURES = {
    'keep_area_tables': [_i32, _i32, _i32, _vp, _vp, _vp],
    'keep_resize_area_u8': [_vp, _vp, _i32, _i32, _i32, _i32, _i32, _vp, _vp, _vp, _vp, _vp, _vp, _vp],
    'keep_resize_linear_u8': [_vp, _vp, _i32, _i32, _i32, _i32, _i32, _vp],
    'keep_resize_linear_fxy_u8': [_vp, _vp, _i32, _i32, _i32, _i32, _i32, C.c_double, C.c_double, _vp],
    'keep_warp_batch_group': [_i32, _i32, _vp, _vp],
    'keep_warp_affine_batch_u8': [_vp, _i32, _i32, _i32, _vp, _i32, _i32, _i32, _vp, _vp, _i32, _i32, _i32, _vp],
    'keep_warp_affine_batch_scatter_u8': [_vp, _i32, _i32, _i32, _vp, _i32, _i32, _i32, _i32, _vp, _vp, _vp, _i32, _i32, _i32, _vp],
    'keep_attention_plan': [C.POINTER(AttnArgs), C.POINTER(AttnPlanOut)],
    'keep_conv2d_launch_plan': [C.POINTER(ConvArgs), C.POINTER(ConvLaunchPlanOut)],
    'keep_gm_ffn_x1_plan': [_i32, _i32, _i32, _i32, _i32],
    'keep_gm_ffn_x1': [_vp, _vp, _vp, _f32, _vp, _f32, _vp, _vp, _f32, _vp, _i64, _i32, _i32, _i32, _vp],
    'keep_frame_signature_u8': [_vp, _i32, _i32, _i32, _vp, _vp],
    'keep_paste_face_w': [_vp, _i32, _i32, _vp, _vp, _i32, _i32, _vp, _i32, _i32, _i32, _i32, _i32, _f32, _vp],
    'keep_tone_match_u8': [_vp, _vp, _vp, _vp, _i32, _i32, _i32, _vp, _i32, _vp],
}
CV_EXPORTED_SYMBOLS = ['keep_cv_abi_version'] + list(_CV_SIGNATURES)

_lib = None
_device_checked = set()


EINVAL, EUNSUP = -1, -2


class KeepHipError(RuntimeError):

    def __init__(self, msg, code=None):
        super().__init__(msg)
        self.code = code


def load(check_device=True):
    global _lib
    if _lib is None:
        if not os.path.exists(LIB_PATH):
            raise KeepHipError(
                f"{LIB_PATH} not found: build it with `python __graft_entry__.py` (hipcc --offload-arch=gfx950). "
                f"There is no CPU/PyTorch fallback for the KEEP hot path.")
        lib = C.CDLL(LIB_PATH)
        lib.keep_abi_version.restype = _i32
        lib.keep_last_error.restype = C.c_char_p
        lib.keep_device_ok.restype = _i32
        lib.keep_device_ok.argtypes = [_i32]
        lib.keep_attention_workspace_bytes.restype = _i64
        lib.keep_attention_workspace_bytes.argtypes = [C.POINTER(AttnArgs)]
        ver = lib.keep_abi_version()
        if ver != ABI_VERSION:
            raise KeepHipError(f"libkeep_hip.so ABI version {ver} != expected {ABI_VERSION}; rebuild")
        lib.keep_sizeof_conv2d_args.restype = lib.keep_sizeof_attention_args.restype = _i32
        for name, struct in (('keep_sizeof_conv2d_args', ConvArgs), ('keep_sizeof_attention_args', AttnArgs)):
            want = getattr(lib, name)()
            if want != C.sizeof(struct):
                raise KeepHipError(f"{name}() = {want} but the ctypes {struct.__name__} is {C.sizeof(struct)} bytes; "
                                   f"engine/hiplib.py and include/keep_hip.h disagree")
        if not hasattr(lib, 'keep_cv_abi_version'):
            raise KeepHipError("libkeep_hip.so lacks the include/keep_cv_hip.h entry points (keep_cv_abi_version); rebuild")
        lib.keep_cv_abi_version.restype = _i32
        ver = lib.keep_cv_abi_version()
        if ver != CV_ABI_VERSION:
            raise KeepHipError(f"libkeep_hip.so keep_cv_hip.h version {ver} != expected {CV_ABI_VERSION}; rebuild")
        for name, argtypes in list(_SIGNATURES.items()) + list(_CV_SIGNATURES.items()):
            fn = getattr(lib, name)
            fn.restype = _i32
            fn.argtypes = argtypes
        _lib = lib
    if check_device:
        dev = torch.cuda.current_device() if torch.cuda.is_available() else None
        if dev is None:
            raise KeepHipError("no HIP device visible: the KEEP hot path runs on MI355X (gfx950) only")
        if dev not in _device_checked:
            rc = _lib.keep_device_ok(dev)
            if rc != 0:
                raise KeepHipError(_lib.keep_last_error().decode(), code=rc)
            _device_checked.add(dev)
    return _lib


def _ptr(t):
    return None if t is None else t.data_ptr()


def _stream():
    return torch.cuda.current_stream().cuda_stream


def _check(rc, what):
    if rc != 0:
        raise KeepHipError(f"{what} failed (code {rc}): {_lib.keep_last_error().decode()}", code=rc)


def call(name, *args):
    lib = load()
    conv = [(_ptr(a) if isinstance(a, torch.Tensor) or a is None else a) for a in args]
    _check(getattr(lib, name)(*conv, _stream()), name)


def conv_args(**kw):
    a = ConvArgs()
    a.struct_size = C.sizeof(ConvArgs)
    for k, v in kw.items():
        setattr(a, k, _ptr(v) if (isinstance(v, torch.Tensor) or v is None) else v)
    return a


def conv2d_plan(a):
    lib = load(check_device=False)
    out = ConvPlanOut()
    _check(lib.keep_conv2d_plan(C.byref(a), C.byref(out)), 'keep_conv2d_plan')
    return out


def conv2d_launch_plan(a):
    lib = load(check_device=False)
    out = ConvLaunchPlanOut()
    _check(lib.keep_conv2d_launch_plan(C.byref(a), C.byref(out)), 'keep_conv2d_launch_plan')
    return out.kernels.decode()


def attention_workspace_bytes(a):
    return int(load(check_device=False).keep_attention_workspace_bytes(C.byref(a)))


def attention_plan(a):
    lib = load(check_device=False)
    out = AttnPlanOut()
    _check(lib.keep_attention_plan(C.byref(a), C.byref(out)), 'keep_attention_plan')
    return out


def attn_args(**kw):
    a = AttnArgs()
    a.struct_size = C.sizeof(AttnArgs)
    for k, v in kw.items():
        setattr(a, k, _ptr(v) if (isinstance(v, torch.Tensor) or v is None) else v)
    return a


def attention_x1_plan(**kw):
    a = attn_args(**dict(kw, mma=MMA_X1, flags=int(kw.get('flags', 0)) | ATTN_X1))
    need = attention_workspace_bytes(a)
    if need < 0:
        raise KeepHipError(f"keep_attention plan failed (code -2): {_lib.keep_last_error().decode()}", code=EUNSUP)
    return need


def gm_ffn_x1_plan(C_, hidden, io_misalign=0, weight_misalign=0, ln_misalign=0):
    lib = load(check_device=False)
    _check(lib.keep_gm_ffn_x1_plan(int(C_), int(hidden), int(io_misalign), int(weight_misalign), int(ln_misalign)), 'keep_gm_ffn_x1_plan')
    return True


def conv2d_launch(a):
    _check(load().keep_conv2d(C.byref(a), _stream()), 'keep_conv2d')


def conv2d(**kw):
    conv2d_launch(conv_args(**kw))


def attention(**kw):
    lib = load()
    a = attn_args(**kw)
    need = int(lib.keep_attention_workspace_bytes(C.byref(a)))
    if need > 0:
        ws = torch.empty((need + 3) // 4, dtype=torch.float32, device=kw['q'].device)
        a.workspace, a.workspace_bytes = ws.data_ptr(), need
    _check(lib.keep_attention(C.byref(a), _stream()), 'keep_attention')
```

comfyui-keep_amd/engine/net.py:

```python
import math
import os

import numpy as np
import torch

from . import hiplib as L
from . import ops
from .arch import (CHANNELS, DEFAULT_ARCH, FUSE_ENCODER_BLOCK, FUSE_GENERATOR_BLOCK, GMFLOW, encoder_blocks,
                   generator_blocks)
from .weights import logical_tensors, pack_blob, validate_state_dict, views

_KNOWN_KW = set(DEFAULT_ARCH) | {
    'gumbel_straight_through', 'gumbel_kl_weight', 'vqgan_path', 'fix_modules', 'flownet_path', 'cfa_nlayers',
    'cross_residual', 'mask_ratio'}


FUSED_GM_MLP = os.environ.get('KEEP_NO_FUSED_MLP') is None
FUSED_GM_FFN_X3 = os.environ.get('KEEP_X3_FUSED_FFN', '1') != '0'
GM_S2D_CONV1 = os.environ.get('KEEP_GM_S2D', '1') != '0'
GM_DEDUP_L0 = os.environ.get('KEEP_GM_DEDUP_L0', '1') != '0'
CHECK_X3_RANGE = os.environ.get('KEEP_X3_NO_RANGE_CHECK') is None
GRAPH_MAX_CLIPS = int(os.environ.get('KEEP_AMD_GRAPH_MAX_CLIPS', '2'))
STREAM_OVERLAP_MAX_CLIPS = int(os.environ.get('KEEP_AMD_OVERLAP_MAX_CLIPS', '2'))
CFT_SPLIT = os.environ.get('KEEP_CFT_SPLIT', '1') != '0'
# ... 602 lines not shown
        g = self.o.linear(m.view(BT * Ltok, C), w['kalman_filter.kalman_gain_calculator.3.weight'],
                       w['kalman_filter.kalman_gain_calculator.3.bias'], act=L.ACT_SIGMOID, n_img=BT)
        return g.view(BT, Ltok)

    def _gm_consts(self, h8, w8, dev):
        key = ('gm', h8, w8, str(dev))
        if key not in self._const:
            C = GMFLOW['feature_channels']
            wh, ww = h8 // 2, w8 // 2
            npf = C // 2
            ye = torch.arange(1, wh + 1, dtype=torch.float32).view(wh, 1).expand(wh, ww)
            xe = torch.arange(1, ww + 1, dtype=torch.float32).view(1, ww).expand(wh, ww)
            eps, sc = 1e-6, 2 * math.pi
            ye = ye / (float(wh) + eps) * sc
            xe = xe / (float(ww) + eps) * sc
            dim_t = torch.arange(npf, dtype=torch.float32)
            dim_t = 10000.0 ** (2 * (dim_t // 2) / npf)
            px = xe[:, :, None] / dim_t
            py = ye[:, :, None] / dim_t
            px = torch.stack((px[:, :, 0::2].sin(), px[:, :, 1::2].cos()), dim=3).flatten(2)
            py = torch.stack((py[:, :, 0::2].sin(), py[:, :, 1::2].cos()), dim=3).flatten(2)
            win = torch.cat((py, px), dim=2)
            table = win.repeat(2, 2, 1).contiguous()
            gy, gx = torch.meshgrid(torch.arange(h8), torch.arange(w8), indexing='ij')
            grid = torch.stack([gx, gy], dim=-1).float().reshape(h8 * w8, 2).contiguous()
            self._const[key] = (table.to(dev), grid.to(dev))
        return self._const[key]

    def _inorm(self, x, st=None):
        return ops.norm_affine(x, None, None, x.shape[-1], 1e-5, stats=st)

    def _gm_resblock(self, x, p, stride):
        w = self.w
        c1, st1 = self.of.conv(x, w[f'{p}.conv1.weight'], None, stride=stride, pad=1, stats=True, bounded=True)
        c2, st2 = self.of.conv(c1, w[f'{p}.conv2.weight'], None, pro=self._inorm(c1, st1), pro_act=L.PRO_RELU, stats=True)
        s2, h2 = self._inorm(c2, st2)
        N, H, Wd, C = c2.shape
        out = torch.empty_like(c2)
        if f'{p}.downsample.0.weight' in w:
            d, std = self.of.conv(x, w[f'{p}.downsample.0.weight'].view(C, 1, 1, -1), w[f'{p}.downsample.0.bias'],
                                 stride=stride, pad=0, ksize=1, stats=True, bounded=True)
            sd, hd = self._inorm(d, std)
            L.call('keep_gm_join', d, sd, hd, c2, s2, h2, out, N, H * Wd, C)
        else:
            L.call('keep_gm_join', x, None, None, c2, s2, h2, out, N, H * Wd, C)
        return out

    def _gm_layer(self, src, tgt, p, ffn, h8, w8, shift, kv_rot, n_img):
        w = self.w
        C = src.shape[-1]
        Ltok = h8 * w8
        wqkv = w[f'{p}.qkv.weight']
        o = torch.empty_like(src)
        if tgt is src:
            qkv = self.of.linear(src, wqkv, out_bf16=True, bounded=True, n_img=n_img)
            q, k, v = qkv, ops.offset(qkv, C), ops.offset(qkv, 2 * C)
            sq = skv = (Ltok * 3 * C, 3 * C, 0)
        else:
            q = self.of.linear(src, wqkv[:C], out_bf16=True, bounded=True, n_img=n_img)
            kv = self.of.linear(tgt, wqkv[C:], out_bf16=True, bounded=True, n_img=n_img)
            k, v = kv, ops.offset(kv, C)
            sq, skv = (Ltok * C, C, 0), (Ltok * 2 * C, 2 * C, 0)
        self.of.attention(q, k, v, o, B=n_img * 4, H=1, Lq=Ltok // 4, Lk=Ltok // 4, D=C, Dv=C, scale=1.0 / (C ** 0.5),
                      q_str=sq, k_str=skv, v_str=skv, o_str=(Ltok * C, C, 0), mode=2, img_h=h8, img_w=w8, ksplit=2,
                      shift=shift, kv_rot=kv_rot, n_img=n_img)
        n1 = (w[f'{p}.norm1.weight'], w[f'{p}.norm1.bias'], 1e-5)
        fuse = self.of.ln_fusable(w[f'{p}.merge.weight'], Ltok)
        if not ffn:
            if fuse:
                return self.of.linear(o, w[f'{p}.merge.weight'], bounded=True, n_img=n_img, ln=n1, residual=src)
            m = self.of.linear(o, w[f'{p}.merge.weight'], bounded=True, n_img=n_img)
            return ops.layernorm(m, n1[0], n1[1], res=src)
        if fuse:
            m = self.of.linear(o, w[f'{p}.merge.weight'], bounded=True, n_img=n_img, ln=n1)
        else:
            m = ops.layernorm(self.of.linear(o, w[f'{p}.merge.weight'], bounded=True, n_img=n_img), n1[0], n1[1])
        if (self.o.mma == L.MMA_X3 and C == 128 and FUSED_GM_FFN_X3 and self.o.x3_twin(w[f'{p}.mlp.0.weight']) is not None):
            return self.o.gm_ffn(src, m, w[f'{p}.mlp.0.weight'], w[f'{p}.mlp.2.weight'], w[f'{p}.norm2.weight'], w[f'{p}.norm2.bias'], 1e-5)
        if self.o.mma == L.MMA_BF16 and C == 128 and FUSED_GM_MLP:
            m2 = self.o.gm_mlp(src, m, w[f'{p}.mlp.0.weight'], w[f'{p}.mlp.2.weight'])
        else:
            if self.o.mma == L.MMA_X3:
                hmid = self.of.linear(src, w[f'{p}.mlp.0.weight'], act=L.ACT_GELU, bounded=True, x2=m, n_img=n_img)
            else:
                hmid = self.of.linear(ops.concat2(src, m), w[f'{p}.mlp.0.weight'], act=L.ACT_GELU, bounded=True, n_img=n_img)
            if self.of.ln_fusable(w[f'{p}.mlp.2.weight'], Ltok):
                return self.of.linear(hmid, w[f'{p}.mlp.2.weight'], bounded=True, n_img=n_img, residual=src,
                                     ln=(w[f'{p}.norm2.weight'], w[f'{p}.norm2.bias'], 1e-5))
            m2 = self.of.linear(hmid, w[f'{p}.mlp.2.weight'], bounded=True, n_img=n_img)
        return ops.layernorm(m2, w[f'{p}.norm2.weight'], w[f'{p}.norm2.bias'], res=src)

    def _gm_backbone(self, img_nchw):
        w = self.w
        pfx = 'flownet.model'
        ws2d = w.get(f'{pfx}.backbone.conv1.weight_s2d') if GM_S2D_CONV1 else None
        if ws2d is not None and img_nchw.shape[2] % 2 == 0 and img_nchw.shape[3] % 2 == 0:
            img = ops.rgb_s2d(img_nchw.contiguous())
            f, fst = self.of.conv(img, ws2d, None, stride=1, pad=2, ksize=4, stats=True, bounded=True, out_hw=img.shape[1:3])
        else:
            img = ops.nchw_to_nhwc(img_nchw, mode=1)
            f, fst = self.of.conv(img, w[f'{pfx}.backbone.conv1.weight'], None, stride=2, pad=3, ksize=7, stats=True)
        s, hh = self._inorm(f, fst)
        x = torch.empty_like(f)
        L.call('keep_affine_act', f, s, hh, x, f.shape[0], f.shape[1] * f.shape[2], f.shape[3], L.ACT_RELU)
        for li, stride in ((1, 1), (2, 2), (3, 2)):
            x = self._gm_resblock(x, f'{pfx}.backbone.layer{li}.0', stride)
            x = self._gm_resblock(x, f'{pfx}.backbone.layer{li}.1', 1)
        return self.of.linear(x, w[f'{pfx}.backbone.conv2.weight'], w[f'{pfx}.backbone.conv2.bias'], bounded=True)

    def _gmflow(self, im1, im2):
        P = im1.shape[0]
        return self._gmflow_pairs(self._gm_backbone(torch.cat([im1, im2], dim=0)), P)

    def _gmflow_clip(self, x):
        B, T = x.shape[:2]
        feat = self._gm_backbone(x.reshape(B * T, *x.shape[2:]))
        key = ('pairs', B, T, str(feat.device))
        if key not in self._const:
# ... 574 lines not shown
```

comfyui-keep_amd/engine/ops.py:

```python
import bisect
import os

import torch

from . import hiplib as L

TOKEN_LINEAR = os.environ.get('KEEP_NO_TOKEN_LINEAR') is None
UP2_PHASES = os.environ.get('KEEP_X3_UP2', '1') != '0'
FUSE_LN = os.environ.get('KEEP_X3_FUSE_LN', '1') != '0'
USE_BK256 = bool(int(os.environ.get('KEEP_BK256', '0')))
HALO_PRENORM_MINPIX = int(os.environ.get('KEEP_HALO_PRENORM_MINPIX', '0'))

DEBUG_SYNC = os.environ.get('KEEP_DEBUG_SYNC') is not None
X3_STREAM_KERNEL = 'conv3x3_halo_x3s_kernel'
X1_UP2_KERNEL = 'conv3x3_halo_x3_kernel<32, x2 phases, true>'
_PLAN_CACHE = {}
POLICY_NAMES = {L.MMA_F32: 'fp32', L.MMA_BF16: 'bf16', L.MMA_X3: 'x3'}
PLAN_REF_IMAGES = int(os.environ.get('KEEP_PLAN_REF_IMAGES', '0') or 0)
DEFAULT_CONV_FLAGS = L.CONV_X3_EXACT_ACT if os.environ.get('KEEP_X3_EXACT_ACT') else 0


class Plan:
    __slots__ = ('split_k', 'ws_floats', 'stats_P', 'wants_bf16_input', 'out_bf16_ok', 'out_amax_ok', 'kernel')

    def __init__(self, o):
        self.split_k = o.split_k
        self.ws_floats = o.workspace_bytes // 4
        self.stats_P = o.stats_P
        self.wants_bf16_input = bool(o.wants_bf16_input)
        self.out_bf16_ok = bool(o.out_bf16_ok)
        self.out_amax_ok = bool(o.out_amax_ok)
        self.kernel = o.kernel.decode()


class Stats:
    __slots__ = ('part', 'P', 'amax')

    def __init__(self, part=None, P=0, amax=None):
        self.part, self.P, self.amax = part, P, amax


def _plan(a, key):
    pl = _PLAN_CACHE.get(key)
    if pl is None:
        pl = _PLAN_CACHE[key] = Plan(L.conv2d_plan(a))
    return pl


def _row_of(table, off, n):
    starts, rows = table
    i = bisect.bisect_right(starts, off) - 1
    return rows[i] if i >= 0 and off + n <= rows[i][1] else None


def empty(shape, like):
    return torch.empty(shape, dtype=torch.float32, device=like.device)


def offset(t, off):
    return t.view(-1)[off:] if off else t


class Ops:
    def __init__(self):
        self.mma = L.MMA_F32
        self.attn_mma = L.MMA_F32
        self.blob32 = None
        self.blob16 = None
        self.blobx3 = None
        self.x3_acc_scale = 1.0
        self._x3_table = None
        self._up2, self._up2_src = {}, (None, None)
        self.profile = None
        self.amax_arena = None
        self.amax_pos = 0
        self.status = None
        self.arena_generation = 0
        self.flags = DEFAULT_CONV_FLAGS
        self.attn_flags = 0
        self.plan_ref_images = PLAN_REF_IMAGES
        self.blobx1 = None
        self._x1_table = None
        self._x1_route, self._up2_x1_route, self._attn_x1_route = {}, {}, {}
        self.x1_flags = L.CONV_X1_GEMM
        self.x1_base = L.MMA_X3
        self.x1_base_kernel = None
        self.census = None
        self.attn_x1 = False
        self.up2_x1 = False
        self.ffn_x1 = False
        self._ffn_x1_route = {}

    def begin_forward(self, device):
        self.ensure_arena(device)
        self._block.zero_()
        self.amax_pos = 0

    def ensure_arena(self, device):
        device = torch.device(device)
        if self.amax_arena is None or self.amax_arena.device != device:
            self._block = torch.empty((1 << 18) + 4, dtype=torch.float32, device=device)
            self.amax_arena = self._block[4:]
            self.status = self._block[:1].view(torch.int32)
            self.arena_generation += 1

    def set_precision(self, mma, blob32=None, blob16=None, blobx3=None, x3_acc_scale=1.0, x3_scales=None):
        if mma not in (L.MMA_F32, L.MMA_BF16, L.MMA_X3):
            raise ValueError(f"set_precision: {mma!r} is no base policy (single fp16 is a base policy plus set_x1_twin)")
        self._x3_table = ([a for a, _, _ in x3_scales], list(x3_scales)) if x3_scales else None
        self.mma = self.attn_mma = mma
        self.set_x1_twin()
        self._forget_routes(self._x1_route, self._up2_x1_route, self._attn_x1_route, self._ffn_x1_route)
        if blobx3 is not None and (blob32 is not self._up2_src[0] or blobx3 is not self._up2_src[1]):
            self._up2, self._up2_src = {}, (blob32, blobx3)
        self.blob32, self.blob16, self.blobx3, self.x3_acc_scale = blob32, blob16, blobx3, float(x3_acc_scale)

    def set_x1_twin(self, blobx1=None, ranges=None, flags=L.CONV_X1_GEMM, base=L.MMA_X3, base_kernel=None):
        if blobx1 is not None and self.mma != base:
            raise ValueError(f"set_x1_twin: this twin rides on the {POLICY_NAMES[base]} policy (set_precision(...) with it first)")
        self.blobx1, self.x1_flags, self.x1_base, self.x1_base_kernel = blobx1, int(flags), base, base_kernel
        self._x1_table = None
        if blobx1 is not None:
            rows = sorted((int(a), int(b), float(s)) for a, b, s in ranges)
            self._x1_table = ([a for a, _, _ in rows], rows)
        self._forget_routes(self._x1_route)

    def _x1_of(self, w):
        if self.blobx1 is None or not w.is_contiguous():
            return None
        off = (w.data_ptr() - self.blob32.data_ptr()) // 4
        row = _row_of(self._x1_table, off, w.numel())
        return None if row is None else (self.blobx1[off:off + w.numel()], row[2])

    def x1_twin(self, w):
        tw = self._x1_of(w)
        return None if tw is None else tw[0]

    @staticmethod
    def _route(routes, key, query):
        r = routes.get(key)
        if r is None:
            try:
                r = query()
            except L.KeepHipError as e:
                if e.code != L.EUNSUP:
                    raise
                r = False
            routes[key] = r
        return r

    @staticmethod
    def _forget_routes(*routes):
        for r in routes:
            r.clear()

    def _blob_off(self, w):
        if self.blob32 is None:
            raise RuntimeError("this precision policy needs the packed weight blobs registered (Ops.set_precision)")
        off = (w.data_ptr() - self.blob32.data_ptr()) // 4
        if off < 0 or off + w.numel() > self.blob32.numel() or not w.is_contiguous():
            raise RuntimeError("weight view is not inside the packed blob; pass the twin explicitly")
        return off

    def bf16_twin(self, w):
        if self.blob16 is None:
# ... 58 lines not shown
        tw = self._up2.get(key)
        if tw is None:
            wp = ffn_w2_perm(w2)
            sc = x3_scale_for(float(wp.abs().max()))
            tw = self._up2[key] = ((wp * sc).to(torch.float16).view(torch.int16).view(-1), 1.0 / sc)
        return tw

    def gm_ffn(self, src, msg, w0, w2, gamma, beta, eps):
        if not self.ffn_x1:
            return self.gm_ffn_x3(src, msg, w0, w2, gamma, beta, eps)
        C = src.shape[-1]
        M = src.numel() // C
        Hd = w0.shape[0]
        out = empty((M, C), src)
        w0x, asc0 = self.ffn_w0_x1_twin(w0)
        w2x, asc2 = self.ffn_w2_x1_twin(w2)

        def mis(*ts):
            r = 0
            for t in ts:
                r |= t.data_ptr() % 16
            return r
        key = (C, Hd, mis(src, msg, out), mis(w0x, w2x), mis(gamma, beta))
        if not self._route(self._ffn_x1_route, key, lambda: L.gm_ffn_x1_plan(*key)):
            return self.gm_ffn_x3(src, msg, w0, w2, gamma, beta, eps)
        if self.profile is not None:
            e0, e1 = torch.cuda.Event(enable_timing=True), torch.cuda.Event(enable_timing=True)
            self.profile.append(('gm_ffn_x1_kernel', 2.0 * M * (2 * C * Hd + Hd * C), 1, e0, e1,
                                 3 * M * C * 4 + (2 * C * Hd + Hd * C) * 2, (M // 4096 if M % 4096 == 0 else 1, M, 1, 2 * C, C, 1, 1, 0, False)))
            e0.record()
        L.call('keep_gm_ffn_x1', src, msg, w0x, float(asc0), w2x, float(asc2), gamma, beta, float(eps), out,
               M, C, Hd, 1 if (self.flags & L.CONV_X3_EXACT_ACT) else 0)
        if self.profile is not None:
            self.profile[-1][4].record()
        return out.view(src.shape)

    def x3_twin(self, w):
        if self.blobx3 is None or w.shape[-1] % 16:
            return None
        off = self._blob_off(w)
        return self.blobx3[2 * off:2 * (off + w.numel())]

    def x3_scale_of(self, w):
        if self._x3_table is None:
            return self.x3_acc_scale
        row = _row_of(self._x3_table, self._blob_off(w), w.numel())
        if row is None:
            raise RuntimeError("weight view does not lie inside one tensor of the x3 blob")
        return row[2]

    def conv(self, x, w, bias=None, *, stride=1, pad=1, ksize=3, down=False, upsample=False, pro=None, pro_act=L.PRO_NONE,
             act=L.ACT_NONE, residual=None, aux=None, aux_w=1.0, cin=None, in_off=0, out=None, split_k=None, wb=None,
             wx3=None, x3_acc_scale=None, mma=None, stats=False, out_bf16=False, bounded=False, x_amax=None, x2=None,
             reflect=False, out_ld=None, ln=None, out_hw=None):
        N, H, W, ld = x.shape
        Cout = w.shape[0]
        Cin = ld if cin is None else cin
        if x2 is not None:
            assert bounded and pro is None and cin is None and in_off == 0, 'x2 needs a bounded, unsliced, prologue-free input'
            Cin = ld + x2.shape[-1]
        KH = KW = ksize
        assert w.numel() == Cout * KH * KW * Cin, (w.shape, Cout, KH, KW, Cin)
        Hv, Wv = (2 * H, 2 * W) if upsample else (H, W)
        if down:
            stride, pad_t, pad_l = 2, 0, 0
            Ho, Wo = Hv // 2, Wv // 2
        else:
            pad_t = pad_l = pad
            Ho = (Hv + 2 * pad - KH) // stride + 1
            Wo = (Wv + 2 * pad - KW) // stride + 1
        if out_hw is not None:
            assert out_hw[0] <= Ho and out_hw[1] <= Wo
            Ho, Wo = out_hw
        M = N * Ho * Wo
        mma = self.mma if mma is None else mma
        in_dtype = L.BF16 if x.dtype == torch.bfloat16 else L.F32
        if mma == L.MMA_BF16 and wb is None and self.blob16 is not None:
            wb = self.bf16_twin(w)
        up_mode = L.UPSAMPLE_X2_PHASES if upsample == L.UPSAMPLE_X2_PHASES and upsample is not True else int(bool(upsample))
        own_up2 = False
        if (upsample and mma == L.MMA_X3 and wx3 is None and UP2_PHASES and KH == 3 and stride == 1 and pad == 1 and not down
                and pro is None and pro_act == L.PRO_NONE and act == L.ACT_NONE and aux is None and x2 is None and not reflect
                and split_k in (None, 1) and H % 8 == 0 and W % 32 == 0 and Cin % 16 == 0 and Cout % 64 == 0 and in_dtype == L.F32
                and not out_bf16 and self.x3_twin(w) is not None):
            wx3, x3_acc_scale = self.up2_twin(w)
            up_mode = L.UPSAMPLE_X2_PHASES
            own_up2 = True
        own_w = wx3 is None
        if mma == L.MMA_X3 and wx3 is None:
            wx3 = self.x3_twin(w)
            if wx3 is not None and x3_acc_scale is None:
                x3_acc_scale = self.x3_scale_of(w)
        if x3_acc_scale is None:
            x3_acc_scale = self.x3_acc_scale
        want_bf16_out = bool(out_bf16) and mma == L.MMA_BF16 and residual is None
        xin = x if in_off == 0 else x.view(-1)[in_off:]

        def in_range():
            return x_amax if (x_amax is not None and x_amax.numel() == N) else absmax(xin, N, H * W, Cin, ld, H * W * ld, self)
        probes = pro is None and not bounded
        in_amax = None
        if ((mma == L.MMA_X3 and (wx3 is not None or (Cin <= 3 and KH == 3))) or mma == L.MMA_X1) and probes:
            in_amax = in_range()
        out_ld = (Cout if out is None else out.shape[-1]) if out_ld is None else out_ld
        sk_req = 0 if split_k is None else int(split_k)
        odt = L.BF16 if want_bf16_out else L.F32
        pol = (mma, wx3, float(x3_acc_scale), self.flags)

        def planned(p=None):
            mma, wx3, acc_scale, flags = p or pol
            a = L.conv_args(
                inp=xin, weight=w, bias=bias, out=out, pro_scale=None if pro is None else pro[0],
                pro_shift=None if pro is None else pro[1], residual=residual, aux=aux, workspace=None,
                N=N, H=H, W=W, Cin=Cin, Cout=Cout, KH=KH, KW=KW, stride=stride, pad_t=pad_t, pad_l=pad_l, Ho=Ho, Wo=Wo,
                in_ld=ld, out_ld=out_ld, res_ld=0 if residual is None else residual.shape[-1],
                upsample=up_mode, pro_act=pro_act, epi_act=act, aux_w=float(aux_w), split_k=sk_req, dtype=in_dtype,
                mma=mma, weight_bf16=wb if mma == L.MMA_BF16 else None, stats_out=None, stats_P=0,
                bk256=int(USE_BK256), out_dtype=odt, weight_x3=wx3 if mma in (L.MMA_X3, L.MMA_X1) else None,
                x3_acc_scale=acc_scale, x3_in_amax=in_amax, x3_out_amax=None,
                in2=x2, in2_cin1=0 if x2 is None else ld, pad_mode=L.PAD_REFLECT if reflect else L.PAD_ZERO,
                ln_gamma=None if ln is None else ln[0], ln_beta=None if ln is None else ln[1],
                ln_eps=0.0 if ln is None else float(ln[2]), flags=flags, plan_ref_images=self.plan_ref_images)
            key = (N, H, W, ld, Cin, Cout, KH, stride, pad_t, pad_l, Ho, Wo, out_ld, up_mode, pro_act, act, in_dtype, mma,
                   odt, sk_req, pro is not None, residual is not None, 0 if residual is None else residual.shape[-1],
                   aux is not None, bias is not None, in_off % 8, wx3 is not None, USE_BK256, x2 is not None, bool(reflect),
                   ln is not None, flags, self.plan_ref_images)
            return a, _plan(a, key), key

        a, pl, key = planned()
        if (pl.wants_bf16_input and in_off == 0 and Cin == ld and N * H * W >= HALO_PRENORM_MINPIX):
            x16 = torch.empty((N, H, W, ld), dtype=torch.bfloat16, device=x.device)
            L.call('keep_norm_act_bf16', x, None if pro is None else pro[0], None if pro is None else pro[1], x16,
                   N, H * W, ld, pro_act, in_dtype)
            x = xin = x16
            pro, pro_act, in_dtype = None, L.PRO_NONE, L.BF16
            a, pl, key = planned()
        cand = None
        if own_up2:
            if self.up2_x1 and Cin % 32 == 0:
                cand = (self._up2_x1_route, *self.up2_x1_twin(w), L.CONV_X1_UP2)
        elif (self.blobx1 is not None and own_w and mma == self.mma == self.x1_base and x2 is None
              and (self.x1_base_kernel is None or (pl.kernel == self.x1_base_kernel and pl.split_k == 1))):
            tw1 = self._x1_of(w)
            if tw1 is not None:
                cand = (self._x1_route, *tw1, self.x1_flags)
        if cand is not None:
            x1 = (L.MMA_X1, cand[1], cand[2], self.flags | cand[3])
            pl1 = self._route(cand[0], key, lambda: planned(x1)[1])
            if pl1:
                if in_amax is None and probes:
                    in_amax = in_range()
                pol = x1
                a, pl = planned()[0], pl1
        if want_bf16_out and not pl.out_bf16_ok:
            want_bf16_out, odt = False, L.F32
            a, pl, key = planned()
        if out is None:
            out = torch.empty((N, Ho, Wo, Cout), dtype=torch.bfloat16 if want_bf16_out else torch.float32, device=x.device)
            a.out = out.data_ptr()
        a.split_k = pl.split_k
        ws = empty((pl.ws_floats,), x) if pl.ws_floats else None
        if ws is not None:
            a.workspace = ws.data_ptr()
        st = None
        if stats and ((pl.stats_P and stats != 'amax') or pl.out_amax_ok):
            st = Stats()
            if pl.stats_P and stats != 'amax':
                st.part, st.P = empty((N, pl.stats_P, Cout, 2), x), pl.stats_P
                a.stats_out, a.stats_P = st.part.data_ptr(), pl.stats_P
            if pl.out_amax_ok:
                st.amax, a.x3_out_amax_zeroed = self._amax_slots(N, x)
                a.x3_out_amax = st.amax.data_ptr()
        if self.profile is not None:
            e0, e1 = torch.cuda.Event(enable_timing=True), torch.cuda.Event(enable_timing=True)
            alg_bytes = (N * H * W * Cin * x.element_size() + Cout * KH * KW * Cin * (2 if mma == L.MMA_BF16 else 4)
                         + M * Cout * out.element_size() + (0 if residual is None else M * Cout * 4))
            self.profile.append((pl.kernel, 2.0 * M * Cout * KH * KW * Cin, pl.split_k, e0, e1, alg_bytes,
                                 (N, H, W, Cin, Cout, KH, stride, int(upsample), pro is not None)))
            e0.record()
        if DEBUG_SYNC:
            import sys
            print(f'[keep] {pl.kernel} N={N} H={H} W={W} ld={ld} Cin={Cin} Cout={Cout} k={KH} s={stride} up={int(upsample)} '
                  f'split={pl.split_k} in_off={in_off} pro={pro is not None}/{pro_act} act={act} res={residual is not None} '
                  f'aux={aux is not None} statsP={pl.stats_P if stats else 0}', file=sys.stderr, flush=True)
        if self.census is not None:
            self.census[pl.kernel] = self.census.get(pl.kernel, 0) + 1
        L.conv2d_launch(a)
        if DEBUG_SYNC:
            torch.cuda.synchronize()
            if not bool(torch.isfinite(out.float()).all()):
                import sys
                print(f'[keep] NON-FINITE output of {pl.kernel}; input finite={bool(torch.isfinite(x.float()).all())} '
                      f'absmax={float(x.float().abs().max()):.4g} pro={None if pro is None else [float(t.abs().max()) for t in pro]} '
                      f'res absmax={None if residual is None else float(residual.abs().max())}', file=sys.stderr, flush=True)
        if self.profile is not None:
            self.profile[-1][4].record()
        return (out, st) if stats else out

    def linear(self, x, w, bias=None, *, act=L.ACT_NONE, residual=None, pro=None, pro_act=L.PRO_NONE, cin=None, in_off=0,
               n_img=None, out_bf16=False, bounded=False, x_amax=None, x2=None, ln=None, want_amax=False):
        shp = x.shape
        ld = shp[-1]
        M = x.numel() // ld
        if n_img is None:
            n_img = shp[0] if x.dim() >= 3 else 1
        assert M % n_img == 0, (tuple(shp), n_img)
        if (TOKEN_LINEAR and self.mma == L.MMA_BF16 and ld == 128 and w.shape[0] in (128, 256, 384) and w.shape[-1] == 128
                and M >= 65536 and act == L.ACT_NONE and residual is None and pro is None and pro_act == L.PRO_NONE
                and cin is None and in_off == 0 and x.dtype == torch.float32 and x.is_contiguous()):
            return self.token_linear(x.view(M, ld), w.view(w.shape[0], 128), bias, out_bf16).reshape(*shp[:-1], w.shape[0])
        x4 = x.reshape(n_img, M // n_img, 1, ld)
        x24 = None if x2 is None else x2.reshape(n_img, M // n_img, 1, x2.shape[-1])
        res4 = None if residual is None else residual.reshape(n_img, M // n_img, 1, residual.shape[-1])
        y = self.conv(x4, w, bias, stride=1, pad=0, ksize=1, pro=pro, pro_act=pro_act, act=act, residual=res4, cin=cin,
                      in_off=in_off, out_bf16=out_bf16, bounded=bounded, x_amax=x_amax, x2=x24, ln=ln, stats='amax' if want_amax else False)
        if want_amax:
            y, st = y
            return y.reshape(*shp[:-1], w.shape[0]), (None if st is None else st.amax)
        return y.reshape(*shp[:-1], w.shape[0])

    def ln_fusable(self, w, rows_per_image):
        return (FUSE_LN and self.mma == L.MMA_X3 and w.shape[0] == 128 and w.shape[-1] % 32 == 0 and rows_per_image % 128 == 0
                and self.x3_twin(w) is not None)

    @staticmethod
    def norm_affine(x, gamma, beta, groups, eps, stats=None):
        N, H, W, C = x.shape
        HW = H * W
        scale = empty((N, C), x)
        shift = empty((N, C), x)
        if stats is not None and stats.part is not None:
            L.call('keep_norm_finalize', stats.part, gamma, beta, scale, shift, N, HW, C, groups, stats.P, float(eps))
            return scale, shift
        assert x.dtype == torch.float32, "bf16 activations carry their statistics from the producing conv's epilogue"
        cpg = C // groups
        if ((cpg % 4 == 0 and HW * cpg <= 32768) or HW <= 1024) and C % 4 == 0 and groups >= 2:
            L.call('keep_group_stats', x, gamma, beta, scale, shift, N, HW, C, groups, float(eps))
            return scale, shift
        P = max(1, min(HW // 64, 1024))
        part = empty((N, P, C, 2), x)
        L.call('keep_chan_stats', x, part, N, HW, C, C, P)
        L.call('keep_norm_finalize', part, gamma, beta, scale, shift, N, HW, C, groups, P, float(eps))
        return scale, shift

    @staticmethod
    def layernorm(x, gamma, beta, *, res=None, pos=None, eps=1e-5):
        C = x.shape[-1]
        M = x.numel() // C
        out = torch.empty_like(x)
        out2 = torch.empty_like(x) if pos is not None else None
        L.call('keep_layernorm', x, gamma, beta, res, out, pos, 0 if pos is None else pos.shape[0], out2, M, C, float(eps))
        return out if pos is None else (out, out2)

    @staticmethod
    def geglu(x):
        F = x.shape[-1] // 2
        M = x.numel() // (2 * F)
        out = empty((*x.shape[:-1], F), x)
        L.call('keep_geglu', x, out, M, F)
        return out

    def _amax_slots(self, N, like):
        if self.amax_arena is not None and self.amax_pos + N <= self.amax_arena.numel():
            out = self.amax_arena[self.amax_pos:self.amax_pos + N]
            self.amax_pos += N
            return out, 1
        return torch.empty((N,), dtype=torch.float32, device=like.device), 0

    def layernorm_amax(self, x, gamma, beta, *, n_img, res=None, eps=1e-5):
        C = x.shape[-1]
        M = x.numel() // C
        out = torch.empty_like(x)
        am, zeroed = self._amax_slots(n_img, x)
        L.call('keep_layernorm_amax', x, gamma, beta, res, out, M, C, float(eps), M // n_img, am, zeroed)
        return out, am

    def geglu_amax(self, x, *, n_img):
        F = x.shape[-1] // 2
        M = x.numel() // (2 * F)
        out = empty((*x.shape[:-1], F), x)
        am, zeroed = self._amax_slots(n_img, x)
        L.call('keep_geglu_amax', x, out, n_img, M // n_img, F, am, zeroed)
        return out, am

    def attention(self, q, k, v, o, *, B, H, Lq, Lk, D, Dv, scale, q_str, k_str, v_str, o_str, mode=0, T=0, seg_len=0,
                  img_h=0, img_w=0, ksplit=0, shift=0, kv_rot=0, n_img=0, mma=None, probe=False, amax=None):
        mma = self.attn_mma if mma is None else mma
        in_dtype = L.F32
        if q.dtype == torch.bfloat16:
            assert k.dtype == torch.bfloat16 and v.dtype == torch.bfloat16
            in_dtype, mma = L.BF16, L.MMA_BF16
        elif mma != L.MMA_F32 and (D % 16 or any(s % 4 for s in (*q_str, *k_str))):
            mma = L.MMA_F32
        given = amax
        amax = (None, None, None)
        if given is not None and all(t is not None and t.numel() == B for t in given) and mma == L.MMA_X3 and mode == 0 and in_dtype == L.F32:
            amax = tuple(given)
        elif probe and mma == L.MMA_X3 and mode == 0 and in_dtype == L.F32:
            amax = (absmax(q, B, Lq, H * D, q_str[1], q_str[0], self), absmax(k, B, Lk, H * D, k_str[1], k_str[0], self),
                    absmax(v, B, Lk, H * Dv, v_str[1], v_str[0], self))
        if DEBUG_SYNC:
            import sys
            print(f'[keep] attention mma={mma} in_dtype={in_dtype} B={B} H={H} Lq={Lq} Lk={Lk} D={D} Dv={Dv} mode={mode}',
                  file=sys.stderr, flush=True)
        kw = dict(q=q, k=k, v=v, o=o,
                  q_bs=q_str[0], q_ts=q_str[1], q_hs=q_str[2], k_bs=k_str[0], k_ts=k_str[1], k_hs=k_str[2],
                  v_bs=v_str[0], v_ts=v_str[1], v_hs=v_str[2], o_bs=o_str[0], o_ts=o_str[1], o_hs=o_str[2],
                  B=B, H=H, Lq=Lq, Lk=Lk, D=D, Dv=Dv, scale=float(scale), mode=mode, T=T, seg_len=seg_len,
                  img_h=img_h, img_w=img_w, ksplit=ksplit, shift=shift, kv_rot=kv_rot, n_img=n_img, mma=mma,
                  in_dtype=in_dtype, q_amax=amax[0], k_amax=amax[1], v_amax=amax[2], flags=self.attn_flags)
        if self.attn_x1 and mma == self.attn_mma == L.MMA_X3 and in_dtype == L.F32:
            key = (H, Lq, Lk, D, Dv, mode, ksplit, img_h, img_w, shift, tuple(s % 4 for s in (*q_str, *k_str, *v_str)),
                   tuple(t.data_ptr() % 16 for t in (q, k, v)), amax[0] is not None, self.attn_flags)
            if self._route(self._attn_x1_route, key, lambda: L.attention_x1_plan(**kw) is not None):
                kw.update(mma=L.MMA_X1, flags=self.attn_flags | L.ATTN_X1)
        L.attention(**kw)
        if DEBUG_SYNC:
            torch.cuda.synchronize()
            if not bool(torch.isfinite(o).all()):
                import sys
                print(f'[keep] NON-FINITE attention output; q/k/v absmax {float(q.float().abs().max()):.4g} '
                      f'{float(k.float().abs().max()):.4g} {float(v.float().abs().max()):.4g}', file=sys.stderr, flush=True)
        return o

    def token_linear(self, x, w, bias=None, out_bf16=False):
        K = x.shape[-1]
        M = x.numel() // K
        N = w.shape[0]
        out = torch.empty((M, N), dtype=torch.bfloat16 if out_bf16 else torch.float32, device=x.device)
        L.call('keep_token_linear', x, self.bf16_twin(w), bias, out, M, K, N, L.BF16 if out_bf16 else L.F32)
        return out

    def gm_mlp(self, a, b, w0, w2):
        C = a.shape[-1]
        M = a.numel() // C
        out = empty((M, C), a)
        L.call('keep_gm_mlp', a, b, self.bf16_twin(w0), self.bf16_twin(w2), out, M, C)
        return out


def absmax(x, N, R, C, ld, img_stride, ops=None):
    out, zeroed = (empty((N,), x), 0) if ops is None else ops._amax_slots(N, x)
    L.call('keep_absmax', x, out, N, R, C, ld, img_stride, zeroed)
    return out


def concat2(a, b, pad_to=1):
    C1, C2 = a.shape[-1], b.shape[-1]
    M = a.numel() // C1
    ld = (C1 + C2 + pad_to - 1) // pad_to * pad_to
    out = empty((*a.shape[:-1], ld), a)
    L.call('keep_concat2', a, b, out, M, C1, C2, ld)
    return out


def add_bcast(a, t, alpha=1.0):
    out = torch.empty_like(a)
    L.call('keep_add_bcast', a, t, out, a.numel(), t.numel(), float(alpha))
    return out


def nchw_to_nhwc(x, mode=0):
    N, C, H, W = x.shape
    out = empty((N, H, W, C), x)
    L.call('keep_nchw_to_nhwc', x, out, N, C, H * W, mode)
    return out


def rgb_s2d(x):
    N, C, H, W = x.shape
    assert C == 3 and H % 2 == 0 and W % 2 == 0
    out = empty((N, H // 2, W // 2, 16), x)
    L.call('keep_rgb_s2d', x, out, N, H, W)
    return out


def nhwc_to_nchw(x):
# ... 75 lines not shown
```

include/keep_cv_hip.h:

```cpp
#ifndef KEEP_CV_HIP_H
#define KEEP_CV_HIP_H

#include <stdint.h>

#include "keep_hip.h"

#ifdef __cplusplus
extern "C" {
#endif

#define KEEP_CV_ABI_VERSION 1

int32_t keep_cv_abi_version(void);

int32_t keep_area_tables(int32_t S, int32_t D, int32_t cap, int32_t* start , int32_t* si , float* alpha );
int32_t keep_resize_area_u8(const uint8_t* src, uint8_t* dst, int32_t N, int32_t H, int32_t W, int32_t H2, int32_t W2,
                            const int32_t* xstart, const int32_t* xsi, const float* xalpha, const int32_t* ystart, const int32_t* ysi,
                            const float* yalpha, void* stream);

int32_t keep_resize_linear_u8(const uint8_t* src, uint8_t* dst, int32_t N, int32_t H, int32_t W, int32_t H2, int32_t W2, void* stream);

int32_t keep_resize_linear_fxy_u8(const uint8_t* src, uint8_t* dst, int32_t N, int32_t H, int32_t W, int32_t H2, int32_t W2, double fx,
                                  double fy, void* stream);

int32_t keep_warp_batch_group(int32_t F, int32_t g, int32_t* first, int32_t* count);
int32_t keep_warp_affine_batch_u8(const uint8_t* frames, int32_t N, int32_t H, int32_t W, uint8_t* dst, int32_t F, int32_t dh, int32_t dw,
                                  const int32_t* frame_of , const double* dst_to_src , int32_t border_b,
                                  int32_t border_g, int32_t border_r, void* stream);
int32_t keep_warp_affine_batch_scatter_u8(const uint8_t* frames, int32_t N, int32_t H, int32_t W, uint8_t* dst, int32_t n_slots, int32_t F,
                                          int32_t dh, int32_t dw, const int32_t* frame_of , const int32_t* slot_of ,
                                          const double* dst_to_src , int32_t border_b, int32_t border_g, int32_t border_r,
                                          void* stream);

typedef struct {
  int32_t waves, dvt, nslices;
  int32_t masked;
  int32_t win_tables;
  int64_t lds_bytes, scratch_bytes;
  char kernel[96];
} keep_attention_plan_out;
int32_t keep_attention_plan(const keep_attention_args* a, keep_attention_plan_out* out);

typedef struct {
  int32_t n_kernels;
  char kernels[508];
} keep_conv2d_launch_plan_out;
int32_t keep_conv2d_launch_plan(const keep_conv2d_args* a, keep_conv2d_launch_plan_out* out);

int32_t keep_gm_ffn_x1_plan(int32_t C, int32_t hidden, int32_t io_misalign, int32_t weight_misalign, int32_t ln_misalign);
int32_t keep_gm_ffn_x1(const float* src, const float* msg, const void* w0_x1, float w0_acc_scale, const void* w2p_x1, float w2_acc_scale,
                       const float* ln_gamma, const float* ln_beta, float ln_eps, float* out, int64_t M, int32_t C, int32_t hidden,
                       int32_t exact_act, void* stream);

int32_t keep_frame_signature_u8(const uint8_t* frames , int32_t N, int32_t H, int32_t W,
                                int32_t* sig , void* stream);

int32_t keep_paste_face_w(float* frame , int32_t H, int32_t W, const uint8_t* face ,
                          const float* mask , int32_t fh, int32_t fw, const double* dst_to_src , int32_t x0, int32_t y0,
                          int32_t x1, int32_t y1, int32_t mask_border, float opacity, void* stream);

int32_t keep_tone_match_u8(const uint8_t* src, const uint8_t* rst, uint8_t* out, int16_t* scratch, int32_t F, int32_t h, int32_t w,
                           const int16_t* taps , int32_t R, void* stream);

#ifdef __cplusplus
}
#endif
#endif
```

Measured before the change: 293.8 frames/s.

## Have the K/V projection GEMM write split-fp16 halves and add a pre-split attention kernel

```diff
diff --git a/comfyui-keep_amd/csrc/keep_attn.hip b/comfyui-keep_amd/csrc/keep_attn.hip
--- a/comfyui-keep_amd/csrc/keep_attn.hip
+++ b/comfyui-keep_amd/csrc/keep_attn.hip
@@ -38,6 +38,7 @@
   ATTN_X3_NQ16,
   ATTN_X3_NQ0,
   ATTN_X3_PACKED,
+  ATTN_X3_PRESPLIT,
   ATTN_X1_PACKED,
   ATTN_X3_SMALL,
   ATTN_X3_TWO_PASS,
@@ -560,10 +561,17 @@
 typedef _Float16 af16x8 __attribute__((ext_vector_type(8)));
 typedef _Float16 af16x4 __attribute__((ext_vector_type(4)));
 typedef _Float16 af16x2 __attribute__((ext_vector_type(2)));
-
-template <int WAVES, int DVT, int NQ, bool PACKED = false, bool X1 = false>
-__global__ __launch_bounds__(64 * WAVES, ((WAVES == 4 && NQ != 16) ? 2 : 1)) void attn_x3_kernel(AttnP p) {
+typedef short as16x4 __attribute__((ext_vector_type(4)));
+typedef unsigned int au32x4 __attribute__((ext_vector_type(4)));
+
+__device__ __forceinline__ af16x4 lds_tr_read(const char* lds) {
+  return __builtin_bit_cast(af16x4, __builtin_amdgcn_ds_read_tr16_b64_v4i16((__attribute__((address_space(3))) as16x4*)lds));
+}
+
+template <int WAVES, int DVT, int NQ, bool PACKED, bool X1, bool KVS>
+__device__ __forceinline__ void attn_x3_body(const AttnP p) {
   static_assert(!X1 || (PACKED && WAVES == 4 && NQ == 8), "the single-fp16 form exists for the packed D = 128 kernel only");
+  static_assert(!KVS || (PACKED && !X1 && WAVES == 4 && NQ == 8 && DVT == 4), "the pre-split form exists for the packed D = Dv = 128 kernel only");
   constexpr bool QREG = NQ > 0;
   constexpr int NQA = QREG ? NQ : 1;
   extern __shared__ __attribute__((aligned(16))) _Float16 smemx[];
@@ -761,9 +769,18 @@
   constexpr int PKK = PACKED ? 32 * ((X1 ? 1 : 2) * 16 * NQA + 8) / 8 : 1;
   constexpr int PKV = PACKED ? DVS * VP / 8 : 1;
   constexpr int PK16 = PKK + PKV;
-  constexpr int PKN = PACKED ? (PK16 + NT - 1) / NT : 1;
+  constexpr int PKN = (PACKED && !KVS) ? (PK16 + NT - 1) / NT : 1;
   uint4 preg[PKN];
+  au32x4 kq[KVS ? 4 : 1], vq[KVS ? 4 : 1];
   auto pk_issue = [&](int kt) {
+    if constexpr (KVS) {
+      const au32x4* kb = reinterpret_cast<const au32x4*>(p.k + (long)wc.img_kv * p.k_bs + kh) + (tid & 31);
+      const au32x4* vb = reinterpret_cast<const au32x4*>(p.v + (long)wc.img_kv * p.v_bs + vh) + ((tid >> 7) << 4) + (((tid >> 5) & 3) << 2) + (tid & 3);
+#pragma unroll
+      for (int u = 0; u < 4; ++u) kq[u] = kb[(long)tpix[kt * 32 + (tid >> 5) + 8 * u] * (p.k_ts >> 2)];
+#pragma unroll
+      for (int u = 0; u < 4; ++u) vq[u] = vb[(long)tpix[kt * 32 + 8 * u + ((tid >> 2) & 7)] * (p.v_ts >> 2)];
+    } else {
     const long tile = ((long)b * p.H + head) * ((p.Lk + 31) >> 5) + kt;
     const uint4* src = reinterpret_cast<const uint4*>(p.kv_pack) + tile * (PKK + p.nslices * PKV);
     const int vs = PKK + (dv0 / DVS) * PKV;
@@ -773,14 +790,33 @@
       preg[u] = make_uint4(0u, 0u, 0u, 0u);
       if (i < PK16) preg[u] = src[i < PKK ? i : vs + (i - PKK)];
     }
+    }
   };
   auto pk_commit = [&]() {
-#pragma unroll
-    for (int u = 0; u < PKN; ++u) {
-      const int i = tid + u * NT;
-      if (i < PK16) reinterpret_cast<uint4*>(Ks)[i] = preg[u];
-    }
-  };
+    if constexpr (KVS) {
+      const int r7 = (tid >> 2) & 7;
+      char* vimg = reinterpret_cast<char*>(Vt) + (tid >> 7) * 8192 + ((tid >> 5) & 3) * 512 + r7 * 64;
+#pragma unroll
+      for (int u = 0; u < 4; ++u) {
+        reinterpret_cast<au32x4*>(Ks)[((tid >> 5) + 8 * u) * (PKK / 32) + (tid & 31)] = kq[u];
+        *reinterpret_cast<au32x4*>(vimg + u * 2048 + 16 * ((tid & 3) ^ (((u & 1) << 1) | (r7 >> 2)))) = vq[u];
+      }
+    } else {
+#pragma unroll
+      for (int u = 0; u < PKN; ++u) {
+        const int i = tid + u * NT;
+        if (i < PK16) reinterpret_cast<uint4*>(Ks)[i] = preg[u];
+      }
+    }
+  };
+  [[maybe_unused]] const char* vtr0 = reinterpret_cast<const char*>(Vt);
+  [[maybe_unused]] const char* vtr1 = vtr0;
+  if constexpr (KVS) {
+    const int q = (lane >> 2) & 3, pp = lane & 3, gg = (lane >> 4) & 1;
+    const int ro = 64 * (4 * lhi + q) + 8 * (pp & 1), cx = 2 * gg + (pp >> 1);
+    vtr0 += ro + 16 * (cx ^ lhi);
+    vtr1 += 2048 + ro + 16 * (cx ^ (2 | lhi));
+  }
 
   const int my_q = q0 + wave * 32 + l31;
   af16x8 qfh[NQA], qfl[NQA];
@@ -939,6 +975,15 @@
       }
 #pragma unroll
       for (int j = 0; j < DVT; ++j) {
+        if constexpr (KVS) {
+          const int vo = 4096 * st + 512 * j;
+          const af16x8 vh8 = __builtin_shufflevector(lds_tr_read(vtr0 + vo), lds_tr_read(vtr1 + vo), 0, 1, 2, 3, 4, 5, 6, 7);
+          const af16x8 vl8 = __builtin_shufflevector(lds_tr_read(vtr0 + 8192 + vo), lds_tr_read(vtr1 + 8192 + vo), 0, 1, 2, 3, 4, 5, 6, 7);
+          o[j] = __builtin_amdgcn_mfma_f32_32x32x16_f16(pl, vh8, o[j], 0, 0, 0);
+          o[j] = __builtin_amdgcn_mfma_f32_32x32x16_f16(ph, vl8, o[j], 0, 0, 0);
+          o[j] = __builtin_amdgcn_mfma_f32_32x32x16_f16(ph, vh8, o[j], 0, 0, 0);
+          continue;
+        }
         const _Float16* vrow = Vt + (j * 32 + l31) * VP + (st * 2 + lhi) * 8;
         const af16x8 vh8 = *reinterpret_cast<const af16x8*>(vrow);
         if (!X1) {
@@ -980,6 +1025,13 @@
     }
   }
 }
+
+template <int WAVES, int DVT, int NQ, bool PACKED = false, bool X1 = false>
+__global__ __launch_bounds__(64 * WAVES, ((WAVES == 4 && NQ != 16) ? 2 : 1)) void attn_x3_kernel(AttnP p) {
+  attn_x3_body<WAVES, DVT, NQ, PACKED, X1, false>(p);
+}
+
+__global__ __launch_bounds__(256, 2) void attn_x3_presplit_kernel(AttnP p) { attn_x3_body<4, 4, 8, true, false, true>(p); }
 
 template <int DC, int DVS, bool X1 = false>
 __global__ __launch_bounds__(256) void attn_pack_kv_x3_kernel(AttnP p, _Float16* out) {
@@ -1055,6 +1107,15 @@
   dim3 grid(cdiv(p.Lq, 128), p.H * p.nslices, p.B);
   hipLaunchKernelGGL((attn_x3_kernel<4, DVT, NQ, true, X1>), grid, dim3(256), pl.lds, st, p);
   KEEP_LAUNCH_CHECK("keep_attention(x3 packed)");
+  return KEEP_OK;
+}
+
+static int launch_attn_x3_presplit(const AttnP& p, const AttnPlan& pl, hipStream_t st) {
+  const int rc = keep_raise_lds_limit<attn_x3_presplit_kernel>("keep_attention");
+  if (rc != KEEP_OK) return rc;
+  dim3 grid(p.Lq / 128, p.nslices, p.B);
+  hipLaunchKernelGGL(attn_x3_presplit_kernel, grid, dim3(256), pl.lds, st, p);
+  KEEP_LAUNCH_CHECK("keep_attention(x3 pre-split)");
   return KEEP_OK;
 }
 
@@ -2123,7 +2184,7 @@
   return KEEP_OK;
 }
 
-static int plan_attention(const keep_attention_args& a, int64_t scratch_avail, AttnP& p, AttnPlan& pl) {
+static int plan_attention(const keep_attention_args& a, int64_t scratch_avail, AttnP& p, AttnPlan& pl, bool kv_split = false) {
   KEEP_REQUIRE(a.B > 0 && a.H > 0 && a.Lq > 0 && a.Lk > 0 && a.D > 0 && a.Dv > 0, "keep_attention: bad dims");
   KEEP_REQUIRE(a.D % 2 == 0 && (a.D <= 128 || a.D % 128 == 0), "keep_attention: D=%d must be even and (<= 128 or a multiple of 128)", a.D);
   KEEP_REQUIRE(a.mode >= 0 && a.mode <= 2, "keep_attention: bad mode %d", a.mode);
@@ -2176,6 +2237,23 @@
   const size_t ntl = (size_t)(a.Lk + 31) / 32;
   const size_t win_tables = ntl * 32 * 4 + ntl * 16 + ntl * 32;
 
+  if (kv_split) {
+    const bool ok = a.mma == KEEP_MMA_X3 && a.in_dtype == KEEP_F32 && a.mode == 2 && a.D == 128 && a.Dv == 128 && a.H == 1 && a.Lq % 128 == 0 &&
+                    a.Lk % 32 == 0 && a.Lk <= 4096 && !a.q_amax && !(a.flags & KEEP_ATTN_NO_X3) && rows16(a.q, a.q_bs, a.q_ts, a.q_hs, 4) &&
+                    rows16(a.k, a.k_bs, a.k_ts, 0, 128) && rows16(a.v, a.v_bs, a.v_ts, 0, 128);
+    if (!ok) {
+      keep_set_error("keep_attention_kv_split: kv_split (k / v as the projection GEMM's split-fp16 halves) needs KEEP_MMA_X3 on fp32 tensors, mode 2, "
+                     "D = Dv = 128, H = 1, Lq %% 128 == 0, Lk %% 32 == 0, Lk <= 4096, no range probes, 16-byte aligned q rows and k / v "
+                     "strides that are multiples of 128");
+      return KEEP_EUNSUP;
+    }
+    pl.form = ATTN_X3_PRESPLIT;
+    pl.waves = 4;
+    pl.nq = 8;
+    pl.win_tables = true;
+    pl.lds = (size_t)(32 * (2 * 128 + 8) + 128 * 72) * 2 + win_tables;
+    return KEEP_OK;
+  }
   if (x1) {
     ATTN_X1_ADMITS(a.in_dtype == KEEP_F32, "keep_attention: KEEP_MMA_X1 needs fp32 q / k / v (in_dtype KEEP_F32)");
     ATTN_X1_ADMITS(a.mode == 0 || a.mode == 2, "keep_attention: KEEP_MMA_X1 covers mode 0 and mode 2, not mode %d", a.mode);
@@ -2302,6 +2380,7 @@
     case ATTN_X3_PACKED:
       snprintf(out, n, "attn_pack_kv_x3_kernel<%d, %d, false> + attn_x3_kernel<4, %d, %d, true, false>", 16 * pl.nq, dvs, pl.dvt, pl.nq);
       return;
+    case ATTN_X3_PRESPLIT: snprintf(out, n, "attn_x3_presplit_kernel"); return;
     case ATTN_X1_PACKED:
       snprintf(out, n, "attn_pack_kv_x3_kernel<%d, %d, true> + attn_x3_kernel<4, %d, %d, true, true>", 16 * pl.nq, dvs, pl.dvt, pl.nq);
       return;
@@ -2313,7 +2392,7 @@
   snprintf(out, n, "?");
 }
 
-extern "C" int32_t keep_attention_plan(const keep_attention_args* a_in, keep_attention_plan_out* out) {
+static int attention_plan_out(const keep_attention_args* a_in, bool kv_split, keep_attention_plan_out* out) {
   KEEP_REQUIRE(out != nullptr, "keep_attention_plan: null out");
   memset(out, 0, sizeof(*out));
   keep_attention_args a;
@@ -2322,7 +2401,7 @@
   AttnP p;
   AttnPlan pl;
   const bool ws_ok = a.workspace && (uintptr_t)a.workspace % 16 == 0;
-  const int rc = plan_attention(a, ws_ok ? a.workspace_bytes : 0, p, pl);
+  const int rc = plan_attention(a, ws_ok ? a.workspace_bytes : 0, p, pl, kv_split);
   if (rc != KEEP_OK) return rc;
   out->waves = pl.waves;
   out->dvt = pl.dvt;
@@ -2332,12 +2411,20 @@
   out->lds_bytes = (int64_t)pl.lds;
   AttnP p_all;
   AttnPlan pl_all;
-  out->scratch_bytes = plan_attention(a, INT64_MAX, p_all, pl_all) == KEEP_OK ? pl_all.scratch : 0;
+  out->scratch_bytes = plan_attention(a, INT64_MAX, p_all, pl_all, kv_split) == KEEP_OK ? pl_all.scratch : 0;
   attn_plan_kernel_name(pl, out->kernel, sizeof(out->kernel));
   return KEEP_OK;
 }
 
-extern "C" int32_t keep_attention(const keep_attention_args* a_in, void* stream) {
+extern "C" int32_t keep_attention_plan(const keep_attention_args* a_in, keep_attention_plan_out* out) {
+  return attention_plan_out(a_in, false, out);
+}
+
+extern "C" int32_t keep_attention_kv_split_plan(const keep_attention_args* a_in, keep_attention_plan_out* out) {
+  return attention_plan_out(a_in, true, out);
+}
+
+static int attention_launch(const keep_attention_args* a_in, bool kv_split, void* stream) {
   keep_attention_args a;
   const int rc_in = attn_args_in(a_in, a);
   if (rc_in != KEEP_OK) return rc_in;
@@ -2345,7 +2432,7 @@
   AttnP p;
   AttnPlan pl;
   const bool ws_ok = a.workspace && (uintptr_t)a.workspace % 16 == 0;
-  const int rc = plan_attention(a, ws_ok ? a.workspace_bytes : 0, p, pl);
+  const int rc = plan_attention(a, ws_ok ? a.workspace_bytes : 0, p, pl, kv_split);
   if (rc != KEEP_OK) return rc;
   hipStream_t st = (hipStream_t)stream;
   const bool one_wave = pl.waves == 1;
@@ -2373,6 +2460,8 @@
       return with_dvt(pl.dvt, [&](auto dvt) {
         return pl.nq == 8 ? launch_attn_x3_packed<decltype(dvt)::value, 8>(p, pl, st) : launch_attn_x3_packed<decltype(dvt)::value, 16>(p, pl, st);
       });
+    case ATTN_X3_PRESPLIT:
+      return launch_attn_x3_presplit(p, pl, st);
     case ATTN_X1_PACKED:
       p.kv_pack = (const _Float16*)a.workspace;
       return launch_attn_x3_packed<4, 8, true>(p, pl, st);
@@ -2388,6 +2477,10 @@
   keep_set_error("keep_attention: no kernel form planned");
   return KEEP_EINVAL;
 }
+
+extern "C" int32_t keep_attention(const keep_attention_args* a_in, void* stream) { return attention_launch(a_in, false, stream); }
+
+extern "C" int32_t keep_attention_kv_split(const keep_attention_args* a_in, void* stream) { return attention_launch(a_in, true, stream); }
 
 #define MLP_C 128
 __global__ __launch_bounds__(256, 2) void gm_mlp_kernel(const float* __restrict__ xa, const float* __restrict__ xb,
diff --git a/comfyui-keep_amd/csrc/keep_conv.hip b/comfyui-keep_amd/csrc/keep_conv.hip
--- a/comfyui-keep_amd/csrc/keep_conv.hip
+++ b/comfyui-keep_amd/csrc/keep_conv.hip
@@ -1629,6 +1629,7 @@
   p.ln_beta = a->ln_beta;
   p.ln_eps = a->ln_eps;
   p.kslice_steps = 0;
+  p.split_c0 = p.split_c1 = 0;
   p.bias = a->bias;
   p.out = (float*)a->out;
   p.pro_scale = a->pro_scale;
@@ -1972,11 +1973,29 @@
   return plan_f32(a, p, g, pl);
 }
 
-static int plan_conv(const keep_conv2d_args* a, ConvP& p, ConvPlan& pl) {
+struct ConvSplit {
+  int c0, c1;
+};
+
+static int plan_conv(const keep_conv2d_args* a, ConvP& p, ConvPlan& pl, ConvSplit sp) {
   memset(&pl, 0, sizeof(pl));
   fill_conv_params(a, p);
   pl.wide = (a->Ho % 8 == 0 && a->Wo % 32 == 0);
   const int rc = plan_form(a, p, conv_geom(a), pl);
+  if (rc == KEEP_OK && (sp.c0 || sp.c1)) {
+    const bool ok = a->mma == KEEP_MMA_X3 && pl.path == PATH_GATHER_X3 && pl.form == FORM_X3_GATHER && pl.gemm && pl.plain && pl.split_k == 1 &&
+                    a->out_dtype == KEEP_F32 && a->epi_act == KEEP_ACT_NONE && !a->residual && !a->aux && !a->stats_out && !a->ln_gamma &&
+                    a->Cout % 128 == 0 && a->out_ld % 128 == 0 && sp.c0 >= 0 && sp.c0 < sp.c1 && sp.c1 <= a->Cout &&
+                    sp.c0 % 128 == 0 && sp.c1 % 128 == 0 && p.M % 128 == 0 && (long)a->out_ld * 4 * 128 < (1L << 30);
+    if (!ok) {
+      keep_set_error("keep_conv2d_split: split_c0 / split_c1 (split-fp16 output columns) need the KEEP_MMA_X3 GEMM form (1x1, stride 1, no prologue / "
+                     "activation / residual / aux / split-K / statistics / LayerNorm), fp32 output, Cout, out_ld and both bounds multiples of 128 "
+                     "and N*Ho*Wo %% 128 == 0");
+      return KEEP_EUNSUP;
+    }
+    p.split_c0 = sp.c0;
+    p.split_c1 = sp.c1;
+  }
   if (rc == KEEP_OK) plan_kernel_name(a, pl);
   return rc;
 }
@@ -1996,7 +2015,7 @@
 
 extern "C" int32_t keep_sizeof_conv2d_args(void) { return (int32_t)sizeof(keep_conv2d_args); }
 
-static int conv_prelude(const keep_conv2d_args* a_in, bool launch, keep_conv2d_args& a, ConvP& p, ConvPlan& pl) {
+static int conv_prelude(const keep_conv2d_args* a_in, bool launch, keep_conv2d_args& a, ConvP& p, ConvPlan& pl, ConvSplit sp = {0, 0}) {
   int rc = conv_args_in(a_in, a);
   if (rc != KEEP_OK) return rc;
   rc = validate_conv(&a);
@@ -2007,15 +2026,15 @@
     KEEP_REQUIRE(!a.pro_scale || ((uintptr_t)a.pro_scale % 16 == 0 && (uintptr_t)a.pro_shift % 16 == 0),
                  "keep_conv2d: pro_scale/pro_shift must be 16-byte aligned");
   }
-  return plan_conv(&a, p, pl);
-}
-
-extern "C" int32_t keep_conv2d_plan(const keep_conv2d_args* a_in, keep_conv2d_plan_out* out) {
+  return plan_conv(&a, p, pl, sp);
+}
+
+static int conv_plan_out(const keep_conv2d_args* a_in, ConvSplit sp, keep_conv2d_plan_out* out) {
   KEEP_REQUIRE(out != nullptr, "keep_conv2d_plan: null output");
   keep_conv2d_args a_local;
   ConvP p;
   ConvPlan pl;
-  const int rc = conv_prelude(a_in, false, a_local, p, pl);
+  const int rc = conv_prelude(a_in, false, a_local, p, pl, sp);
   if (rc != KEEP_OK) return rc;
   const keep_conv2d_args* a = &a_local;
   memset(out, 0, sizeof(*out));
@@ -2032,6 +2051,13 @@
   return KEEP_OK;
 }
 
+extern "C" int32_t keep_conv2d_plan(const keep_conv2d_args* a_in, keep_conv2d_plan_out* out) { return conv_plan_out(a_in, {0, 0}, out); }
+
+extern "C" int32_t keep_conv2d_split_plan(const keep_conv2d_args* a_in, int32_t split_c0, int32_t split_c1, keep_conv2d_plan_out* out) {
+  KEEP_REQUIRE(split_c0 || split_c1, "keep_conv2d_split: empty column range");
+  return conv_plan_out(a_in, {split_c0, split_c1}, out);
+}
+
 void keep_conv_trace_add(ConvTrace* tr, const char* mangled) {
   int status = 0;
   char* full = abi::__cxa_demangle(mangled, nullptr, nullptr, &status);
@@ -2057,11 +2083,11 @@
   ++tr->count;
 }
 
-static int conv_launch(const keep_conv2d_args* a_in, void* stream, ConvTrace* tr) {
+static int conv_launch(const keep_conv2d_args* a_in, void* stream, ConvTrace* tr, ConvSplit sp = {0, 0}) {
   keep_conv2d_args a_local;
   ConvP p;
   ConvPlan pl;
-  int rc = conv_prelude(a_in, true, a_local, p, pl);
+  int rc = conv_prelude(a_in, true, a_local, p, pl, sp);
   if (rc != KEEP_OK) return rc;
   const keep_conv2d_args* a = &a_local;
   if (pl.path == PATH_NEEDS_PRENORM) {
@@ -2236,6 +2262,11 @@
 
 extern "C" int32_t keep_conv2d(const keep_conv2d_args* a_in, void* stream) { return conv_launch(a_in, stream, nullptr); }
 
+extern "C" int32_t keep_conv2d_split(const keep_conv2d_args* a_in, int32_t split_c0, int32_t split_c1, void* stream) {
+  KEEP_REQUIRE(split_c0 || split_c1, "keep_conv2d_split: empty column range");
+  return conv_launch(a_in, stream, nullptr, {split_c0, split_c1});
+}
+
 extern "C" int32_t keep_conv2d_launch_plan(const keep_conv2d_args* a_in, keep_conv2d_launch_plan_out* out) {
   KEEP_REQUIRE(out != nullptr, "keep_conv2d_launch_plan: null output");
   memset(out, 0, sizeof(*out));
diff --git a/comfyui-keep_amd/csrc/keep_conv_common.h b/comfyui-keep_amd/csrc/keep_conv_common.h
--- a/comfyui-keep_amd/csrc/keep_conv_common.h
+++ b/comfyui-keep_amd/csrc/keep_conv_common.h
@@ -54,6 +54,7 @@
   const float* ln_beta;
   float ln_eps;
   int kslice_steps;
+  int split_c0, split_c1;
 };
 
 
diff --git a/comfyui-keep_amd/csrc/keep_conv_x3.hip b/comfyui-keep_amd/csrc/keep_conv_x3.hip
--- a/comfyui-keep_amd/csrc/keep_conv_x3.hip
+++ b/comfyui-keep_amd/csrc/keep_conv_x3.hip
@@ -495,7 +495,8 @@
   const bool cok = co < p.Cout;
   const int row0 = wm * WR + prow;
   const __amdgpu_buffer_rsrc_t out_rsrc = make_rsrc(p.out + m0 * p.out_ld, BM * p.out_ld * 4);
-  const int v_out = cok ? (row0 * p.out_ld + co) * 4 : (int)0x80000000;
+  const bool split = SIMPLE && n0 >= p.split_c0 && n0 < p.split_c1;
+  const int v_out = !cok ? (int)0x80000000 : split ? row0 * p.out_ld * 4 + (co >> 7) * 512 + (co & 127) * 2 : (row0 * p.out_ld + co) * 4;
   __amdgpu_buffer_rsrc_t res_rsrc = out_rsrc, aux_rsrc = out_rsrc, ws_rsrc = out_rsrc;
   int v_res = (int)0x80000000, v_aux = (int)0x80000000, v_ws = (int)0x80000000;
   if (p.res) {
@@ -571,7 +572,16 @@
         for (int q = 0; q < 4; ++q) e[q] += rr[q];
       }
     }
-    {
+    if (SIMPLE && split) {
+      f16x4 h4, l4;
+#pragma unroll
+      for (int q = 0; q < 4; ++q) {
+        h4[q] = (_Float16)e[q];
+        l4[q] = (_Float16)(e[q] - (float)h4[q]);
+      }
+      __builtin_amdgcn_raw_buffer_store_b64(__builtin_bit_cast(u32x2, h4), out_rsrc, v_out + it * RPI * p.out_ld * 4, 0, KEEP_ST_AUX_GEMM);
+      __builtin_amdgcn_raw_buffer_store_b64(__builtin_bit_cast(u32x2, l4), out_rsrc, v_out + it * RPI * p.out_ld * 4 + 256, 0, KEEP_ST_AUX_GEMM);
+    } else {
       u32x4 o;
       o.x = __float_as_uint(e[0]); o.y = __float_as_uint(e[1]); o.z = __float_as_uint(e[2]); o.w = __float_as_uint(e[3]);
       __builtin_amdgcn_raw_buffer_store_b128(o, out_rsrc, v_out + it * RPI * p.out_ld * 4, 0, KEEP_ST_AUX_GEMM);
diff --git a/comfyui-keep_amd/engine/hiplib.py b/comfyui-keep_amd/engine/hiplib.py
--- a/comfyui-keep_amd/engine/hiplib.py
+++ b/comfyui-keep_amd/engine/hiplib.py
@@ -136,6 +136,10 @@
     'keep_frame_signature_u8': [_vp, _i32, _i32, _i32, _vp, _vp],
     'keep_paste_face_w': [_vp, _i32, _i32, _vp, _vp, _i32, _i32, _vp, _i32, _i32, _i32, _i32, _i32, _f32, _vp],
     'keep_tone_match_u8': [_vp, _vp, _vp, _vp, _i32, _i32, _i32, _vp, _i32, _vp],
+    'keep_conv2d_split': [C.POINTER(ConvArgs), _i32, _i32, _vp],
+    'keep_conv2d_split_plan': [C.POINTER(ConvArgs), _i32, _i32, C.POINTER(ConvPlanOut)],
+    'keep_attention_kv_split': [C.POINTER(AttnArgs), _vp],
+    'keep_attention_kv_split_plan': [C.POINTER(AttnArgs), C.POINTER(AttnPlanOut)],
 }
 CV_EXPORTED_SYMBOLS = ['keep_cv_abi_version'] + list(_CV_SIGNATURES)
 
@@ -233,6 +237,13 @@
     return out
 
 
+def conv2d_split_plan(a, split_cols):
+    lib = load(check_device=False)
+    out = ConvPlanOut()
+    _check(lib.keep_conv2d_split_plan(C.byref(a), int(split_cols[0]), int(split_cols[1]), C.byref(out)), 'keep_conv2d_split_plan')
+    return out
+
+
 def conv2d_launch_plan(a):
     lib = load(check_device=False)
     out = ConvLaunchPlanOut()
@@ -244,9 +255,12 @@
     return int(load(check_device=False).keep_attention_workspace_bytes(C.byref(a)))
 
 
-def attention_plan(a):
+def attention_plan(a, kv_split=False):
     lib = load(check_device=False)
     out = AttnPlanOut()
+    if kv_split:
+        _check(lib.keep_attention_kv_split_plan(C.byref(a), C.byref(out)), 'keep_attention_kv_split_plan')
+        return out
     _check(lib.keep_attention_plan(C.byref(a), C.byref(out)), 'keep_attention_plan')
     return out
 
@@ -277,13 +291,20 @@
     _check(load().keep_conv2d(C.byref(a), _stream()), 'keep_conv2d')
 
 
+def conv2d_split_launch(a, split_cols):
+    _check(load().keep_conv2d_split(C.byref(a), int(split_cols[0]), int(split_cols[1]), _stream()), 'keep_conv2d_split')
+
+
 def conv2d(**kw):
     conv2d_launch(conv_args(**kw))
 
 
-def attention(**kw):
+def attention(kv_split=False, **kw):
     lib = load()
     a = attn_args(**kw)
+    if kv_split:
+        _check(lib.keep_attention_kv_split(C.byref(a), _stream()), 'keep_attention_kv_split')
+        return
     need = int(lib.keep_attention_workspace_bytes(C.byref(a)))
     if need > 0:
         ws = torch.empty((need + 3) // 4, dtype=torch.float32, device=kw['q'].device)
diff --git a/comfyui-keep_amd/engine/net.py b/comfyui-keep_amd/engine/net.py
--- a/comfyui-keep_amd/engine/net.py
+++ b/comfyui-keep_amd/engine/net.py
@@ -678,18 +678,21 @@
         Ltok = h8 * w8
         wqkv = w[f'{p}.qkv.weight']
         o = torch.empty_like(src)
+        sq, skv = ((Ltok * 3 * C, 3 * C, 0),) * 2 if tgt is src else ((Ltok * C, C, 0), (Ltok * 2 * C, 2 * C, 0))
+        cols = (C, 3 * C) if tgt is src else (0, 2 * C)
+        split = (self.of.mma == L.MMA_X3 and self.of.x3_twin(wqkv) is not None and
+                 self.of.kv_split_ok(B=n_img * 4, Lq=Ltok // 4, Lk=Ltok // 4, D=C, Dv=C, q_str=sq, k_str=skv, v_str=skv, img_h=h8, img_w=w8,
+                                     ksplit=2, shift=shift, n_img=n_img, gemm=(Ltok, C, cols[1], cols)))
         if tgt is src:
-            qkv = self.of.linear(src, wqkv, out_bf16=True, bounded=True, n_img=n_img)
+            qkv = self.of.linear(src, wqkv, out_bf16=True, bounded=True, n_img=n_img, split_cols=cols if split else None)
             q, k, v = qkv, ops.offset(qkv, C), ops.offset(qkv, 2 * C)
-            sq = skv = (Ltok * 3 * C, 3 * C, 0)
         else:
             q = self.of.linear(src, wqkv[:C], out_bf16=True, bounded=True, n_img=n_img)
-            kv = self.of.linear(tgt, wqkv[C:], out_bf16=True, bounded=True, n_img=n_img)
+            kv = self.of.linear(tgt, wqkv[C:], out_bf16=True, bounded=True, n_img=n_img, split_cols=cols if split else None)
             k, v = kv, ops.offset(kv, C)
-            sq, skv = (Ltok * C, C, 0), (Ltok * 2 * C, 2 * C, 0)
         self.of.attention(q, k, v, o, B=n_img * 4, H=1, Lq=Ltok // 4, Lk=Ltok // 4, D=C, Dv=C, scale=1.0 / (C ** 0.5),
                       q_str=sq, k_str=skv, v_str=skv, o_str=(Ltok * C, C, 0), mode=2, img_h=h8, img_w=w8, ksplit=2,
-                      shift=shift, kv_rot=kv_rot, n_img=n_img)
+                      shift=shift, kv_rot=kv_rot, n_img=n_img, kv_split=split)
         n1 = (w[f'{p}.norm1.weight'], w[f'{p}.norm1.bias'], 1e-5)
         fuse = self.of.ln_fusable(w[f'{p}.merge.weight'], Ltok)
         if not ffn:
diff --git a/comfyui-keep_amd/engine/ops.py b/comfyui-keep_amd/engine/ops.py
--- a/comfyui-keep_amd/engine/ops.py
+++ b/comfyui-keep_amd/engine/ops.py
@@ -7,6 +7,7 @@
 
 TOKEN_LINEAR = os.environ.get('KEEP_NO_TOKEN_LINEAR') is None
 UP2_PHASES = os.environ.get('KEEP_X3_UP2', '1') != '0'
+ATTN_PRESPLIT = os.environ.get('KEEP_X3_ATTN_PRESPLIT', '1') != '0'
 FUSE_LN = os.environ.get('KEEP_X3_FUSE_LN', '1') != '0'
 USE_BK256 = bool(int(os.environ.get('KEEP_BK256', '0')))
 HALO_PRENORM_MINPIX = int(os.environ.get('KEEP_HALO_PRENORM_MINPIX', '0'))
@@ -40,10 +41,10 @@
         self.part, self.P, self.amax = part, P, amax
 
 
-def _plan(a, key):
+def _plan(a, key, split_cols=None):
     pl = _PLAN_CACHE.get(key)
     if pl is None:
-        pl = _PLAN_CACHE[key] = Plan(L.conv2d_plan(a))
+        pl = _PLAN_CACHE[key] = Plan(L.conv2d_plan(a) if split_cols is None else L.conv2d_split_plan(a, split_cols))
     return pl
 
 
@@ -82,6 +83,7 @@
         self.blobx1 = None
         self._x1_table = None
         self._x1_route, self._up2_x1_route, self._attn_x1_route = {}, {}, {}
+        self._kv_split_route = {}
         self.x1_flags = L.CONV_X1_GEMM
         self.x1_base = L.MMA_X3
         self.x1_base_kernel = None
@@ -110,7 +112,7 @@
         self._x3_table = ([a for a, _, _ in x3_scales], list(x3_scales)) if x3_scales else None
         self.mma = self.attn_mma = mma
         self.set_x1_twin()
-        self._forget_routes(self._x1_route, self._up2_x1_route, self._attn_x1_route, self._ffn_x1_route)
+        self._forget_routes(self._x1_route, self._up2_x1_route, self._attn_x1_route, self._ffn_x1_route, self._kv_split_route)
         if blobx3 is not None and (blob32 is not self._up2_src[0] or blobx3 is not self._up2_src[1]):
             self._up2, self._up2_src = {}, (blob32, blobx3)
         self.blob32, self.blob16, self.blobx3, self.x3_acc_scale = blob32, blob16, blobx3, float(x3_acc_scale)
@@ -275,7 +277,7 @@
     def conv(self, x, w, bias=None, *, stride=1, pad=1, ksize=3, down=False, upsample=False, pro=None, pro_act=L.PRO_NONE,
              act=L.ACT_NONE, residual=None, aux=None, aux_w=1.0, cin=None, in_off=0, out=None, split_k=None, wb=None,
              wx3=None, x3_acc_scale=None, mma=None, stats=False, out_bf16=False, bounded=False, x_amax=None, x2=None,
-             reflect=False, out_ld=None, ln=None, out_hw=None):
+             reflect=False, out_ld=None, ln=None, out_hw=None, split_cols=None):
         N, H, W, ld = x.shape
         Cout = w.shape[0]
         Cin = ld if cin is None else cin
@@ -347,8 +349,8 @@
             key = (N, H, W, ld, Cin, Cout, KH, stride, pad_t, pad_l, Ho, Wo, out_ld, up_mode, pro_act, act, in_dtype, mma,
                    odt, sk_req, pro is not None, residual is not None, 0 if residual is None else residual.shape[-1],
                    aux is not None, bias is not None, in_off % 8, wx3 is not None, USE_BK256, x2 is not None, bool(reflect),
-                   ln is not None, flags, self.plan_ref_images)
-            return a, _plan(a, key), key
+                   ln is not None, flags, self.plan_ref_images, None if split_cols is None else tuple(split_cols))
+            return a, _plan(a, key, split_cols), key
 
         a, pl, key = planned()
         if (pl.wants_bf16_input and in_off == 0 and Cin == ld and N * H * W >= HALO_PRENORM_MINPIX):
@@ -408,7 +410,10 @@
                   f'aux={aux is not None} statsP={pl.stats_P if stats else 0}', file=sys.stderr, flush=True)
         if self.census is not None:
             self.census[pl.kernel] = self.census.get(pl.kernel, 0) + 1
-        L.conv2d_launch(a)
+        if split_cols is None:
+            L.conv2d_launch(a)
+        else:
+            L.conv2d_split_launch(a, split_cols)
         if DEBUG_SYNC:
             torch.cuda.synchronize()
             if not bool(torch.isfinite(out.float()).all()):
@@ -421,7 +426,7 @@
         return (out, st) if stats else out
 
     def linear(self, x, w, bias=None, *, act=L.ACT_NONE, residual=None, pro=None, pro_act=L.PRO_NONE, cin=None, in_off=0,
-               n_img=None, out_bf16=False, bounded=False, x_amax=None, x2=None, ln=None, want_amax=False):
+               n_img=None, out_bf16=False, bounded=False, x_amax=None, x2=None, ln=None, want_amax=False, split_cols=None):
         shp = x.shape
         ld = shp[-1]
         M = x.numel() // ld
@@ -429,14 +434,15 @@
             n_img = shp[0] if x.dim() >= 3 else 1
         assert M % n_img == 0, (tuple(shp), n_img)
         if (TOKEN_LINEAR and self.mma == L.MMA_BF16 and ld == 128 and w.shape[0] in (128, 256, 384) and w.shape[-1] == 128
-                and M >= 65536 and act == L.ACT_NONE and residual is None and pro is None and pro_act == L.PRO_NONE
+                and M >= 65536 and act == L.ACT_NONE and residual is None and pro is None and pro_act == L.PRO_NONE and split_cols is None
                 and cin is None and in_off == 0 and x.dtype == torch.float32 and x.is_contiguous()):
             return self.token_linear(x.view(M, ld), w.view(w.shape[0], 128), bias, out_bf16).reshape(*shp[:-1], w.shape[0])
         x4 = x.reshape(n_img, M // n_img, 1, ld)
         x24 = None if x2 is None else x2.reshape(n_img, M // n_img, 1, x2.shape[-1])
         res4 = None if residual is None else residual.reshape(n_img, M // n_img, 1, residual.shape[-1])
         y = self.conv(x4, w, bias, stride=1, pad=0, ksize=1, pro=pro, pro_act=pro_act, act=act, residual=res4, cin=cin,
-                      in_off=in_off, out_bf16=out_bf16, bounded=bounded, x_amax=x_amax, x2=x24, ln=ln, stats='amax' if want_amax else False)
+                      in_off=in_off, out_bf16=out_bf16, bounded=bounded, x_amax=x_amax, x2=x24, ln=ln, stats='amax' if want_amax else False,
+                      split_cols=split_cols)
         if want_amax:
             y, st = y
             return y.reshape(*shp[:-1], w.shape[0]), (None if st is None else st.amax)
@@ -507,7 +513,7 @@
         return out, am
 
     def attention(self, q, k, v, o, *, B, H, Lq, Lk, D, Dv, scale, q_str, k_str, v_str, o_str, mode=0, T=0, seg_len=0,
-                  img_h=0, img_w=0, ksplit=0, shift=0, kv_rot=0, n_img=0, mma=None, probe=False, amax=None):
+                  img_h=0, img_w=0, ksplit=0, shift=0, kv_rot=0, n_img=0, mma=None, probe=False, amax=None, kv_split=False):
         mma = self.attn_mma if mma is None else mma
         in_dtype = L.F32
         if q.dtype == torch.bfloat16:
@@ -532,7 +538,9 @@
                   B=B, H=H, Lq=Lq, Lk=Lk, D=D, Dv=Dv, scale=float(scale), mode=mode, T=T, seg_len=seg_len,
                   img_h=img_h, img_w=img_w, ksplit=ksplit, shift=shift, kv_rot=kv_rot, n_img=n_img, mma=mma,
                   in_dtype=in_dtype, q_amax=amax[0], k_amax=amax[1], v_amax=amax[2], flags=self.attn_flags)
-        if self.attn_x1 and mma == self.attn_mma == L.MMA_X3 and in_dtype == L.F32:
+        if kv_split:
+            kw.update(kv_split=True)
+        elif self.attn_x1 and mma == self.attn_mma == L.MMA_X3 and in_dtype == L.F32:
             key = (H, Lq, Lk, D, Dv, mode, ksplit, img_h, img_w, shift, tuple(s % 4 for s in (*q_str, *k_str, *v_str)),
                    tuple(t.data_ptr() % 16 for t in (q, k, v)), amax[0] is not None, self.attn_flags)
             if self._route(self._attn_x1_route, key, lambda: L.attention_x1_plan(**kw) is not None):
@@ -546,6 +554,27 @@
                       f'{float(k.float().abs().max()):.4g} {float(v.float().abs().max()):.4g}', file=sys.stderr, flush=True)
         return o
 
+    def kv_split_ok(self, *, B, Lq, Lk, D, Dv, q_str, k_str, v_str, img_h, img_w, ksplit, shift, n_img, gemm=None):
+        if not ATTN_PRESPLIT or self.attn_x1 or self.attn_mma != L.MMA_X3:
+            return False
+        key = (Lq, Lk, D, Dv, tuple(q_str), tuple(k_str), tuple(v_str), img_h, img_w, ksplit, shift, self.attn_flags,
+               None if gemm is None else (tuple(gemm[:3]), tuple(gemm[3]), self.mma, self.flags, self.plan_ref_images, USE_BK256))
+
+        def query():
+            a = L.attn_args(q=0x10000, k=0x10000, v=0x10000, o=0x10000, q_bs=q_str[0], q_ts=q_str[1], q_hs=q_str[2], k_bs=k_str[0], k_ts=k_str[1],
+                            k_hs=k_str[2], v_bs=v_str[0], v_ts=v_str[1], v_hs=v_str[2], o_bs=Lq * ksplit * ksplit * Dv, o_ts=Dv, o_hs=0, B=B, H=1,
+                            Lq=Lq, Lk=Lk, D=D, Dv=Dv, scale=1.0, mode=2, img_h=img_h, img_w=img_w, ksplit=ksplit, shift=shift, kv_rot=0,
+                            n_img=n_img, mma=L.MMA_X3, in_dtype=L.F32, flags=self.attn_flags)
+            L.attention_plan(a, kv_split=True)
+            if gemm is not None:
+                rows, cin, cout, cols = gemm
+                g = L.conv_args(inp=0x10000, weight=0x10000, out=0x10000, weight_x3=0x10000, x3_acc_scale=1.0, N=1, H=rows, W=1, Cin=cin, Cout=cout,
+                                KH=1, KW=1, stride=1, Ho=rows, Wo=1, in_ld=cin, out_ld=cout, mma=self.mma, dtype=L.F32, out_dtype=L.F32,
+                                bk256=int(USE_BK256), flags=self.flags, plan_ref_images=self.plan_ref_images)
+                L.conv2d_split_plan(g, cols)
+            return True
+        return self._route(self._kv_split_route, key, query)
+
     def token_linear(self, x, w, bias=None, out_bf16=False):
         K = x.shape[-1]
         M = x.numel() // K
diff --git a/include/keep_cv_hip.h b/include/keep_cv_hip.h
--- a/include/keep_cv_hip.h
+++ b/include/keep_cv_hip.h
@@ -47,6 +47,11 @@
 } keep_conv2d_launch_plan_out;
 int32_t keep_conv2d_launch_plan(const keep_conv2d_args* a, keep_conv2d_launch_plan_out* out);
 
+int32_t keep_conv2d_split(const keep_conv2d_args* a, int32_t split_c0, int32_t split_c1, void* stream);
+int32_t keep_conv2d_split_plan(const keep_conv2d_args* a, int32_t split_c0, int32_t split_c1, keep_conv2d_plan_out* out);
+int32_t keep_attention_kv_split(const keep_attention_args* a, void* stream);
+int32_t keep_attention_kv_split_plan(const keep_attention_args* a, keep_attention_plan_out* out);
+
 int32_t keep_gm_ffn_x1_plan(int32_t C, int32_t hidden, int32_t io_misalign, int32_t weight_misalign, int32_t ln_misalign);
 int32_t keep_gm_ffn_x1(const float* src, const float* msg, const void* w0_x1, float w0_acc_scale, const void* w2p_x1, float w2_acc_scale,
                        const float* ln_gamma, const float* ln_beta, float ln_eps, float* out, int64_t M, int32_t C, int32_t hidden,
```

Result: faster. 297.2 frames/s, median of 6 (+1.2%).
